# LMNS3d/SOFTX_2020_200

Hardware: AMD Instinct MI355X
Metric: nonlinear iters/sec (3D cavity Q2 128^3 BDF2) (higher is better)
Workload: dtype f64; 1 GPU; 3D lid-driven cavity Q2-Q2 128^3 transient BDF2 (BASELINE configs[2]); n_dofs=67898372, n_cells=2097152, parallelism=single

## Files before the change

include/gls_native.h:

```cpp
#ifndef GLS_NATIVE_H
#define GLS_NATIVE_H

#include <stddef.h>
#include <stdint.h>

#ifdef __cplusplus
extern "C" {
#endif

#define GLS_OK 0
#define GLS_EINVAL -1
#define GLS_EHIP -2
#define GLS_ENOMEM -3
#define GLS_ENOCONV -4
#define GLS_EIO -5
#define GLS_ECOMM -6
#define GLS_ENOTFOUND -7

enum gls_scheme {
  GLS_STEADY = 0, GLS_BDF1, GLS_BDF2, GLS_BDF3, GLS_SDIRK2, GLS_SDIRK2_1, GLS_SDIRK2_2,
  GLS_SDIRK3, GLS_SDIRK3_1, GLS_SDIRK3_2, GLS_SDIRK3_3
};

const char *gls_last_error(void);
// ... 9 lines not shown
  const int32_t *cell_vnodes;
  const int32_t *cell_pnodes;
  const double *cell_x0;
  const double *cell_h;
  const uint8_t *vnode_mask;
  double viscosity;
  int srf;
  double omega[3];
  const double *force_q;
  int map_degree;
  const double *cell_support;
} gls_mesh_desc;

typedef struct gls_ctx gls_ctx;

int gls_create(const gls_mesh_desc *desc, gls_ctx **out);
int gls_destroy(gls_ctx *ctx);
int gls_set_stream(gls_ctx *ctx, void *hip_stream);
int gls_n_dofs(const gls_ctx *ctx, int64_t *n_dofs);
int gls_quadrature_points(const gls_ctx *ctx, double *xq);
int gls_uses_brick_kernels(const gls_ctx *ctx);
int gls_set_force(gls_ctx *ctx, const double *force_q);
int gls_set_viscosity(gls_ctx *ctx, double viscosity);

int gls_set_time(gls_ctx *ctx, int scheme, const double time_steps[4]);

int gls_set_state(gls_ctx *ctx, const double *u, const double *u1, const double *u2, const double *u3);

int gls_residual(gls_ctx *ctx, double *rhs);

int gls_jacobian_apply(gls_ctx *ctx, const double *v, double *Jv);

int gls_jacobian_apply_f32(gls_ctx *ctx, const double *v, double *Jv);

int gls_set_hanging(gls_ctx *ctx, int64_t n_lines, const int64_t *dofs, const int64_t *offsets,
                    const int64_t *masters, const double *weights);

int gls_forest_bricks(const gls_ctx *ctx);

int gls_jacobian_diagonal(gls_ctx *ctx, double *diag);

int gls_residual_and_diagonal(gls_ctx *ctx, double *rhs, double *diag);

int gls_set_dirichlet(gls_ctx *ctx, int64_t n, const int64_t *dofs, const double *values);
int gls_apply_dirichlet(gls_ctx *ctx, double *x);

#define GLS_LIN_GMRES 0
#define GLS_LIN_BICGSTAB 1
#define GLS_ORTHO_GRAM 0
#define GLS_ORTHO_CGS2 1
typedef struct {
  int max_iterations;
  int restart;
  double relative_residual, minimum_residual;
  int iterations;
  double final_residual;
  int method;
  int orthogonalization;
  int true_residual;
} gls_linear_params;
int gls_solve_linear(gls_ctx *ctx, const double *rhs, double *x, gls_linear_params *prm);

typedef struct {
  int n_levels;
  gls_ctx **levels;
  int pre_smooth, post_smooth, coarse_sweeps;
  double omega;
  double coarse_omega;
  int coarse_direct;
  int mixed_precision;
  const int *level_sweeps;
  int smoother;
  int smoother_operator;
} gls_mg_params;
int gls_mg_attach(gls_ctx *ctx, const gls_mg_params *prm);
int gls_mg_attach_transfers(gls_ctx *ctx, const gls_mg_params *prm, const int64_t *const *p_off,
                            const int32_t *const *p_col, const double *const *p_w, const int64_t *const *inject);
int gls_mg_attach_replica(gls_ctx *ctx, const gls_mg_params *prm, gls_ctx *replica, const int64_t *p_off,
                          const int32_t *p_col, const double *p_w, const int64_t *inject);
int gls_apply_preconditioner(gls_ctx *ctx, const double *v, double *z);
int gls_mg_smoother_apply(gls_ctx *ctx, const double *v, double *y);
int gls_mg_transfer(gls_ctx *ctx, int level, int direction, const double *in, double *out);
int gls_mg_residual_restrict(gls_ctx *ctx, int level, const double *x, const double *b, double *bc, int *fused);
int gls_set_lattice(gls_ctx *ctx, int n1d, const int64_t *local_to_global);
int gls_mg_detach(gls_ctx *ctx);
int gls_mg_set_coarse_replica(gls_ctx *ctx, gls_ctx *replica, int64_t n_local, const int64_t *local_to_replica);
#define GLS_ILU_MAX_FILL 10
int gls_ilu_attach(gls_ctx *ctx, int fill, double athresh, double rthresh);
int gls_ilu_detach(gls_ctx *ctx);
#define GLS_ILU_ORDER_CM 0
#define GLS_ILU_ORDER_MULTICOLOR 1
int gls_ilu_set_options(gls_ctx *ctx, int ordering, int64_t block_dofs);
int gls_ilu_info(const gls_ctx *ctx, int64_t *nnz, int *n_probes);
int gls_ilu_matrix(gls_ctx *ctx, int32_t *rowp, int32_t *col, double *val);
int gls_ilu_factors(gls_ctx *ctx, int32_t *perm, int32_t *rowp, int32_t *col, double *val);
int gls_iluk_pattern(int64_t n, const int32_t *rowp, const int32_t *col, int fill, int32_t *out_rowp,
                     int32_t *out_col, int32_t *out_level, int64_t capacity, int64_t *out_nnz);
int gls_cuthill_mckee(int64_t n_nodes, const int64_t *adj_off, const int64_t *adj, const int64_t *dof_off,
                      const int64_t *dofs, int64_t *order);

#define GLS_SEC_ASSEMBLE_SYSTEM 0
#define GLS_SEC_ASSEMBLE_RHS 1
#define GLS_SEC_SETUP_ILU 2
#define GLS_SEC_SETUP_GMG 3
#define GLS_SEC_SOLVE_LINEAR 4
#define GLS_N_SECTIONS 5
int gls_section_timing(gls_ctx *ctx, int enable);
int gls_section_get(const gls_ctx *ctx, int section, double *seconds, int *calls);

#define GLS_NEWTON 0
#define GLS_SKIP_NEWTON 1
typedef struct {
  double tolerance;
  int max_iterations;
  int verbosity;
  gls_linear_params lin;
  int newton_iterations;
  int linear_iterations;
  int residual_evaluations;
  double final_residual;
  int solver;
  int skip_iterations;
  int is_initial_step;
  int force_matrix_renewal;
  int linear_failures;
} gls_newton_params;
int gls_freeze_jacobian(gls_ctx *ctx, int freeze);
int gls_newton_solve(gls_ctx *ctx, double *present, const double *u1, const double *u2, const double *u3,
                     gls_newton_params *prm);

typedef struct gls_part gls_part;
int gls_part_create(int n_cells, int nodes_per_cell, const int32_t *cell_vnodes, int n_vnodes, int rank, int world,
                    gls_part **out);
int gls_part_sizes(const gls_part *p, int64_t *cell_begin, int64_t *cell_end, int64_t *n_owned_nodes,
                   int64_t *n_local_nodes, int *n_nbrs, int64_t *n_send, int64_t *n_recv);
int gls_part_get(const gls_part *p, int32_t *local_cell_vnodes, int64_t *local_to_global, int *nbr_ranks,
                 int64_t *send_offsets, int32_t *send_nodes, int64_t *recv_offsets, int32_t *recv_nodes);
int gls_part_destroy(gls_part *p);

typedef int (*gls_exchange_fn)(void *user, int phase);
typedef int (*gls_allreduce_fn)(void *user, double *dev_buf, int n);
#define GLS_RED_BUF_MIN 256
int gls_dist_attach(gls_ctx *ctx, int64_t n_owned_nodes, int n_nbrs, const int64_t *send_offsets,
                    const int32_t *send_nodes, const int64_t *recv_offsets, const int32_t *recv_nodes, double *send_buf,
                    double *recv_buf, double *red_buf, gls_exchange_fn xchg, gls_allreduce_fn allreduce, void *user);
int gls_dist_import(gls_ctx *ctx, double *x);
#define GLS_RCCL_ID_BYTES 128
typedef struct gls_rccl gls_rccl;
int gls_rccl_unique_id(unsigned char *id_out);
int gls_rccl_create(const unsigned char *id, int rank, int world, gls_rccl **out);
int gls_rccl_destroy(gls_rccl *comm);
int gls_rccl_info(const gls_rccl *comm, int *rank, int *world);
int gls_dist_attach_rccl(gls_ctx *ctx, gls_rccl *comm, int64_t n_owned_nodes, int n_nbrs, const int *nbr_ranks,
                         const int64_t *send_offsets, const int32_t *send_nodes, const int64_t *recv_offsets,
                         const int32_t *recv_nodes);

typedef struct gls_gpart gls_gpart;
int gls_gpart_create(int dim, int k, int kp, int64_t n_cells, const int32_t *cell_vnodes, const int32_t *cell_pnodes,
                     int64_t n_vnodes, int64_t n_pnodes, int64_t n_lines, const int64_t *line_dofs,
                     const int64_t *line_offsets, const int64_t *line_masters, int rank, int world, gls_gpart **out);
int gls_gpart_sizes(const gls_gpart *p, int64_t *cell_begin, int64_t *cell_end, int64_t *n_vnodes, int64_t *n_pnodes,
                    int64_t *n_owned_vnodes, int64_t *n_owned_pnodes, int *n_nbrs, int64_t *n_send, int64_t *n_recv);
int gls_gpart_get(const gls_gpart *p, int32_t *local_cell_vnodes, int32_t *local_cell_pnodes, int64_t *vnode_l2g,
                  int64_t *pnode_l2g, int *nbr_ranks, int64_t *send_offsets, int32_t *send_dofs, int64_t *recv_offsets,
                  int32_t *recv_dofs);
int gls_gpart_map_dofs(const gls_gpart *p, int64_t n, const int64_t *global_dofs, int64_t *local_dofs);
// ... 182 lines not shown
```

softx_2020_200_amd/csrc/gls_api.cpp:

```cpp
#include <hip/hip_runtime.h>

#include <algorithm>
#include <array>
#include <chrono>
#include <cmath>
#include <cstdlib>
#include <cstdarg>
#include <cstdio>
#include <cstring>
#include <map>
#include <array>
#include <memory>
#include <string>
#include <vector>
#include <set>
#include <thread>

#include <rocblas/rocblas.h>
#include <rocsolver/rocsolver.h>
#include <rocsparse/rocsparse.h>
#include <rccl/rccl.h>

#include "../../include/gls_native.h"
#include "gls_common.hpp"
// ... 912 lines not shown
  if (c->dist.xchg(c->dist.user, 0) != 0) return set_err(GLS_ECOMM, "ghost import exchange failed");
  HIP_TRY(gls::vec_unpack_nodes(x, c->dist.recv_nodes.p, c->dist.n_recv, voff, c->dist.recv_buf, 0, c->stream));
  return GLS_OK;
}
int upload_export_order(gls_ctx::Dist &D, const int32_t *send, int64_t ns) {
  std::vector<std::pair<int32_t, int32_t>> ds;
  ds.reserve((size_t)ns);
  for (int64_t j = 0; j < ns; ++j) ds.push_back({send[j], (int32_t)j});
  std::stable_sort(ds.begin(), ds.end(), [](const std::pair<int32_t, int32_t> &a, const std::pair<int32_t, int32_t> &b) {
    return a.first < b.first;
  });
  std::vector<int32_t> au, aoff{0}, aslot;
  for (size_t t = 0; t < ds.size(); ++t) {
    if (t == 0 || ds[t].first != ds[t - 1].first) {
      if (t) aoff.push_back((int32_t)aslot.size());
      au.push_back(ds[t].first);
    }
    aslot.push_back(ds[t].second);
  }
  if (!au.empty()) aoff.push_back((int32_t)aslot.size());
  GLS_TRY(D.add_u.upload(au.data(), au.size()));
  GLS_TRY(D.add_off.upload(aoff.data(), au.empty() ? 0 : aoff.size()));
  return D.add_slot.upload(aslot.data(), aslot.size());
}
int dist_export_add(gls_ctx *c, double *y) {
  if (!c->dist.on) return GLS_OK;
  if (c->dist.dofs) {
    HIP_TRY(gls::vec_pack_dofs(y, c->dist.recv_nodes.p, c->dist.n_recv, c->dist.recv_buf, c->stream));
    if (c->dist.xchg(c->dist.user, 1) != 0) return set_err(GLS_ECOMM, "ghost export exchange failed");
    HIP_TRY(gls::vec_add_dofs_ordered(y, c->dist.add_u.p, c->dist.add_off.p, c->dist.add_slot.p, (int64_t)c->dist.add_u.n,
                                      c->dist.send_buf, c->stream));
    return GLS_OK;
  }
  const int64_t voff = 3 * (int64_t)c->n_vnodes;
  HIP_TRY(gls::vec_pack_nodes(y, c->dist.recv_nodes.p, c->dist.n_recv, voff, c->dist.recv_buf, c->stream));
  if (c->dist.xchg(c->dist.user, 1) != 0) return set_err(GLS_ECOMM, "ghost export exchange failed");
  HIP_TRY(gls::vec_add_nodes_ordered(y, c->dist.add_u.p, c->dist.add_off.p, c->dist.add_slot.p, (int64_t)c->dist.add_u.n,
                                     voff, c->dist.send_buf, c->stream));
  return GLS_OK;
}
int dist_multidot(gls_ctx *c, const double *A, int64_t lda, int nk, const double *w, double *host_out) {
  const int64_t n1 = c->dist.on ? (int64_t)c->dim * c->dist.n_owned : c->n_dofs;
  const int64_t off2 = c->dist.on ? (int64_t)c->dim * c->n_vnodes : 0;
  const int64_t n2 = c->dist.on ? c->dist.n_owned_p : 0;
  HIP_TRY(gls::vec_multidot2(A, lda, nk, w, n1, off2, n2, c->scal.p, c->work.p, c->stream));
  if (c->dist.on) {
    HIP_TRY(hipMemcpyAsync(c->dist.red_buf, c->scal.p, sizeof(double) * nk, hipMemcpyDeviceToDevice, c->stream));
    if (c->dist.allreduce(c->dist.user, c->dist.red_buf, nk) != 0) return set_err(GLS_ECOMM, "allreduce failed");
    HIP_TRY(hipMemcpyAsync(host_out, c->dist.red_buf, sizeof(double) * nk, hipMemcpyDeviceToHost, c->stream));
  } else {
    HIP_TRY(hipMemcpyAsync(host_out, c->scal.p, sizeof(double) * nk, hipMemcpyDeviceToHost, c->stream));
  }
  HIP_TRY(hipStreamSynchronize(c->stream));
  return GLS_OK;
}

int lin_f32_target(gls_ctx *c, gls::OpParams &P) {
  P.qdf = nullptr;
  if (!c->smooth_f32 || !gls::brick_fused_jacobi_supported(c->k)) return GLS_OK;
  if (c->qdata32.n != c->qdata.n) GLS_TRY(c->qdata32.alloc(c->qdata.n));
  P.qdf = c->qdata32.p;
  P.oseen = c->smooth_oseen ? 1 : 0;
  return GLS_OK;
}

int ensure_qdata(gls_ctx *c) {
  if (c->qd_valid) return GLS_OK;
  const size_t n = gls::brick_qdata_size(c->k, c->n_cells);
  if (c->qdata.n != n) GLS_TRY(c->qdata.alloc(n));
  gls::OpParams P = make_params(c, true);
  P.qd = c->qdata.p;
  GLS_TRY(lin_f32_target(c, P));
  {
    TimedLaunch t(c, 3);
    HIP_TRY(gls::launch_brick_kernel(c->k, gls::MODE_LIN, P, c->tables, c->stream));
  }
  c->qd_valid = true;
  c->qd32_valid = P.qdf != nullptr;
  c->qd32_partial = P.qdf != nullptr && P.oseen;
  return GLS_OK;
}

hipError_t slab_sum_ex(gls_ctx *g, const double *slab, const float *slabf, double *y, const uint8_t *vmask,
                       const double *jb, const double *jd, double omega, const double *rb, double *x0 = nullptr) {
  if (g->cube_nb1 > 0)
    return gls::brick_slab_sum_cube(g->k, g->cube_nb1, slab, slabf, g->n_vnodes, y, vmask, jb, jd, omega, g->stream, rb,
                                    x0);
  if (x0) return hipErrorInvalidValue;
  return gls::brick_slab_sum_ex(slab, slabf, g->sum_nodes.p, g->sum_off.p, g->sum_slots.p, (int64_t)g->sum_nodes.n,
                                g->n_vnodes, y, vmask, jb, jd, omega, g->stream, rb);
}
hipError_t slab_sum(gls_ctx *c, double *y) {
  if (c->cube_nb1 > 0)
    return gls::brick_slab_sum_cube(c->k, c->cube_nb1, c->slab.p, nullptr, c->n_vnodes, y, nullptr, nullptr, nullptr, 0.0,
                                    c->stream);
  return gls::brick_slab_sum(c->slab.p, c->sum_nodes.p, c->sum_off.p, c->sum_slots.p, (int64_t)c->sum_nodes.n,
                             c->n_vnodes, y, c->stream);
}

int rccl_exchange_on(gls_ctx *c, int phase, hipStream_t stream);

int build_brick_split(gls_ctx *c, const std::vector<char> &flag) {
  const int nvc = gls::ipow(c->k + 1, 3), nb = c->n_cells / 8;
  std::vector<int32_t> cv((size_t)c->n_cells * nvc);
  HIP_TRY(hipMemcpy(cv.data(), c->cell_vnodes.p, cv.size() * sizeof(int32_t), hipMemcpyDeviceToHost));
  std::vector<int32_t> bnd, inn;
  for (int b = 0; b < nb; ++b) {
    bool on = false;
    for (size_t e = (size_t)b * 8 * nvc; e < (size_t)(b + 1) * 8 * nvc && !on; ++e) on = flag[(size_t)cv[e]] != 0;
    (on ? bnd : inn).push_back(b);
  }
  c->split_bnd = (int)bnd.size();
  c->split_int = (int)inn.size();
  bnd.insert(bnd.end(), inn.begin(), inn.end());
  return c->split.upload(bnd.data(), std::max<size_t>(bnd.size(), 1));
}

bool split_jv_enabled(gls_ctx *c) {
  if (!c->use_brick || !c->use_qdata || c->use_colors || c->hang.on || !gls::brick_subset_supported(c->k)) return false;
  if (c->dist.on)
    return c->split.p && (c->dist.comm != nullptr || std::getenv("GLS_SPLIT_DIST"));
  const char *t = std::getenv("GLS_SPLIT_TEST");
  if (!t || std::atoi(t) < 1) return false;
  if (!c->split.p) {
    const int m = std::atoi(t), nb = c->n_cells / 8;
    std::vector<int32_t> bnd, inn;
    for (int b = 0; b < nb; ++b) (b % m == 0 ? bnd : inn).push_back(b);
    c->split_bnd = (int)bnd.size();
    c->split_int = (int)inn.size();
    bnd.insert(bnd.end(), inn.begin(), inn.end());
    if (c->split.upload(bnd.data(), std::max<size_t>(bnd.size(), 1)) != GLS_OK) return false;
  }
  return true;
}

int ensure_element_maps(gls_ctx *c) {
  if (c->ev.p || c->n_cells == 0) return GLS_OK;
  const int dim = c->dim, nv = gls::ipow(c->k + 1, dim), np = gls::ipow(c->kp + 1, dim), el = nv * dim + np;
  std::vector<int32_t> cv((size_t)c->n_cells * nv), cp;
  HIP_TRY(hipMemcpy(cv.data(), c->cell_vnodes.p, cv.size() * sizeof(int32_t), hipMemcpyDeviceToHost));
  if (c->cell_pnodes.p) {
    cp.resize((size_t)c->n_cells * np);
    HIP_TRY(hipMemcpy(cp.data(), c->cell_pnodes.p, cp.size() * sizeof(int32_t), hipMemcpyDeviceToHost));
  }
  const std::vector<int32_t> &pn = c->cell_pnodes.p ? cp : cv;
  std::vector<int64_t> voff((size_t)c->n_vnodes + 1, 0), poff((size_t)c->n_pnodes + 1, 0);
  for (int64_t e = 0; e < (int64_t)c->n_cells * nv; ++e) ++voff[(size_t)cv[(size_t)e] + 1];
  for (int64_t e = 0; e < (int64_t)c->n_cells * np; ++e) ++poff[(size_t)pn[(size_t)e] + 1];
  for (size_t i = 1; i < voff.size(); ++i) voff[i] += voff[i - 1];
  for (size_t i = 1; i < poff.size(); ++i) poff[i] += poff[i - 1];
  std::vector<int64_t> vslot((size_t)voff.back()), pslot((size_t)poff.back());
  std::vector<int64_t> vf(voff.begin(), voff.end() - 1), pf(poff.begin(), poff.end() - 1);
  for (int64_t cell = 0; cell < c->n_cells; ++cell) {
    for (int a = 0; a < nv; ++a) vslot[(size_t)vf[(size_t)cv[(size_t)(cell * nv + a)]]++] = cell * el + (int64_t)a * dim;
    for (int a = 0; a < np; ++a) pslot[(size_t)pf[(size_t)pn[(size_t)(cell * np + a)]]++] = cell * el + (int64_t)nv * dim + a;
  }
  GLS_TRY(c->ev_voff.upload(voff.data(), voff.size()));
  GLS_TRY(c->ev_vslot.upload(vslot.data(), std::max<size_t>(vslot.size(), 1)));
  GLS_TRY(c->ev_poff.upload(poff.data(), poff.size()));
  GLS_TRY(c->ev_pslot.upload(pslot.data(), std::max<size_t>(pslot.size(), 1)));
  return c->ev.alloc((size_t)c->n_cells * el);
}

int ensure_diag(gls_ctx *c);
bool cell_cache_on(const gls_ctx *c) {
  return !c->use_brick && c->n_cells > 0;
}
size_t cell_cache_size(const gls_ctx *c) {
  const int dim = c->dim;
  return (size_t)c->n_cells * (size_t)gls::ipow(c->nq1d, dim) * (size_t)(dim + dim * dim + 1 + dim);
}
// ... 667 lines not shown
  HIP_TRY(gls::vec_gather_scale_set(y, c->diag.p, v, c->con_dofs.p, (int64_t)c->con_dofs.n, c->stream));
  return GLS_OK;
}

namespace {
int ensure_qdata32(gls_ctx *g, bool full = true) {
  GLS_TRY(ensure_qdata(g));
  if (!g->qd32_valid || (full && g->qd32_partial)) {
    if (g->qdata32.n != g->qdata.n) GLS_TRY(g->qdata32.alloc(g->qdata.n));
    HIP_TRY(gls::vec_to_f32(g->qdata.p, g->qdata32.p, (int64_t)g->qdata.n, g->stream));
    g->qd32_valid = true;
    g->qd32_partial = false;
  }
  return GLS_OK;
}
bool slab_f32() { return std::getenv("GLS_SLAB_F64") == nullptr; }
bool first_sweep_fusable(gls_ctx *g) {
  const char *e = std::getenv("GLS_MG_FIRST_FUSE");
  return e && std::atoi(e) != 0 && g->smooth_f32 && g->use_brick && g->use_qdata && !g->use_colors && !g->dist.on &&
         !g->hang.on && g->k == 2 && g->cube_nb1 > 0 && g->use_slab && gls::pencil_enabled() &&
         std::getenv("GLS_MG_NO_FUSE") == nullptr;
}
int jacobian_apply_f32(gls_ctx *g, const double *v, double *y, const double *rb = nullptr, double first_omega = 0.0,
                       bool oseen = false) {
  if (!g->u) return set_err(GLS_EINVAL, "gls_set_state was not called");
  GLS_TRY(ensure_diag(g));
  GLS_TRY(ensure_qdata32(g, !oseen));
  GLS_TRY(dist_import(g, const_cast<double *>(v)));
  gls::OpParams P = make_params(g, true);
  P.qdf = g->qdata32.p;
  P.oseen = oseen ? 1 : 0;
  P.v = v;
  P.y = y;
  const bool col = g->use_colors;
  P.slab = col ? nullptr : brick_slab(g);
  const bool fuse_rb = rb && (P.slab || col) && !g->dist.on && gls::brick_fused_jacobi_supported(g->k) &&
                       std::getenv("GLS_MG_NO_FUSE") == nullptr;
  P.rb = fuse_rb ? rb : nullptr;
  P.slabf = P.slab && slab_f32() && gls::brick_fused_jacobi_supported(g->k) ? reinterpret_cast<float *>(P.slab)
                                                                             : nullptr;
  if (first_omega > 0.0) {
    if (!fuse_rb || !first_sweep_fusable(g)) return set_err(GLS_EINVAL, "fused first sweep not applicable");
    P.jx0 = const_cast<double *>(v);
    P.jd = g->diag.p;
    P.jomega = first_omega;
  }
  if (col) set_colors(g, P, y);
  if (!col && !P.slab) HIP_TRY(hipMemsetAsync(y, 0, sizeof(double) * g->n_dofs, g->stream));
  {
    TimedLaunch t(g, 4);
    HIP_TRY(gls::launch_brick_jv_f32(g->k, P, g->tables, g->stream));
  }
  if (P.slab) {
    TimedLaunch t(g, 5);
    HIP_TRY(slab_sum_ex(g, P.slab, P.slabf, y, nullptr, nullptr, P.jx0 ? g->diag.p : nullptr, P.jomega, P.rb, P.jx0));
  }
  GLS_TRY(dist_export_add(g, y));
  HIP_TRY(gls::vec_gather_scale_set(y, g->diag.p, v, g->con_dofs.p, (int64_t)g->con_dofs.n, g->stream, P.rb));
  if (rb && !fuse_rb) HIP_TRY(gls::vec_axpby(y, 1.0, rb, -1.0, g->n_dofs, g->stream));
  return GLS_OK;
}
int smoother_apply(gls_ctx *g, const double *v, double *y, const double *rb = nullptr) {
  if (g->smooth_f32 && g->use_brick && g->use_qdata) return jacobian_apply_f32(g, v, y, rb, 0.0, g->smooth_oseen);
  g->oct.f32_next = g->smooth_f32 && g->oct.on;
  const int rc = gls_jacobian_apply(g, v, y);
  g->oct.f32_next = false;
  GLS_TRY(rc);
  if (rb) HIP_TRY(gls::vec_axpby(y, 1.0, rb, -1.0, g->n_dofs, g->stream));
  return GLS_OK;
}
}
static int ensure_ilu(gls_ctx *c);
static int ilu_probe(gls_ctx *c);
static int apply_ilu(gls_ctx *c, const double *v, double *z);
namespace {
int ilu_sweep(gls_ctx *g, double *x, const double *b, double *y, double *z) {
  GLS_TRY(ensure_ilu(g));
  GLS_TRY(gls_jacobian_apply(g, x, y));
  HIP_TRY(gls::vec_axpby(y, 1.0, b, -1.0, g->n_dofs, g->stream));
  GLS_TRY(apply_ilu(g, y, z));
  HIP_TRY(gls::vec_axpy(x, 1.0, z, g->n_dofs, g->stream));
  return GLS_OK;
}
int smoother_sweep(gls_ctx *g, double *x, const double *b, double *y, double omega, double *z = nullptr) {
  if (z && g->ilu.on && !g->ilu.probe_only) return ilu_sweep(g, x, b, y, z);
  const bool nofuse = std::getenv("GLS_MG_NO_FUSE") != nullptr;
  const bool brick = g->use_brick && g->use_qdata && (g->use_colors || brick_slab(g)) && !g->dist.on &&
                     !g->hang.on && gls::brick_fused_jacobi_supported(g->k);
  if (nofuse || !brick) {
    GLS_TRY(smoother_apply(g, x, y));
    HIP_TRY(gls::mg_jacobi_update(x, b, y, g->diag.p, omega, g->n_dofs, 0, g->stream));
    return GLS_OK;
  }
  if (!g->u) return set_err(GLS_EINVAL, "gls_set_state was not called");
  GLS_TRY(ensure_diag(g));
  const bool f32 = g->smooth_f32;
  GLS_TRY(f32 ? ensure_qdata32(g, !g->smooth_oseen) : ensure_qdata(g));
  gls::OpParams P = make_params(g, true);
  P.v = x;
  P.y = x;
  P.jx = x;
  P.jb = b;
  P.jd = g->diag.p;
  P.jomega = omega;
  if (g->use_colors) {
    if (g->acc.n != (size_t)g->n_dofs) GLS_TRY(g->acc.alloc((size_t)g->n_dofs));
    set_colors(g, P, g->acc.p);
  } else {
    P.slab = brick_slab(g);
  }
  if (f32) {
    P.qdf = g->qdata32.p;
    P.oseen = g->smooth_oseen ? 1 : 0;
    P.slabf = P.slab && slab_f32() ? reinterpret_cast<float *>(P.slab) : nullptr;
    TimedLaunch t(g, 4);
    HIP_TRY(gls::launch_brick_jv_f32(g->k, P, g->tables, g->stream));
  } else {
    P.qd = g->qdata.p;
    TimedLaunch t(g, 1);
    HIP_TRY(gls::launch_brick_kernel(g->k, gls::MODE_JVQ, P, g->tables, g->stream));
  }
  if (g->use_colors) return GLS_OK;
  TimedLaunch t(g, 5);
  HIP_TRY(slab_sum_ex(g, P.slab, P.slabf, x, g->vmask.p, b, g->diag.p, omega, nullptr));
  return GLS_OK;
}
}

int gls_mg_smoother_apply(gls_ctx *c, const double *v, double *y) {
  GLS_TRY(check_ctx(c));
  if (!v || !y || v == y) return set_err(GLS_EINVAL, "v/y null or aliased");
  return smoother_apply(c, v, y);
}

int gls_jacobian_apply_f32(gls_ctx *c, const double *v, double *y) {
  GLS_TRY(check_ctx(c));
  if (!v || !y || v == y) return set_err(GLS_EINVAL, "v/y null or aliased");
  if (!(c->use_brick && c->use_qdata)) return set_err(GLS_EINVAL, "FP32 J.v needs the 3D Qk-Qk brick path");
  return jacobian_apply_f32(c, v, y);
}

int gls_set_dirichlet(gls_ctx *c, int64_t n, const int64_t *dofs, const double *vals) {
  GLS_TRY(check_ctx(c));
  if (n < 0 || (n > 0 && (!dofs || !vals))) return set_err(GLS_EINVAL, "dirichlet arrays");
  for (int64_t i = 0; i < n; ++i)
    if (dofs[i] < 0 || dofs[i] >= c->n_dofs) return set_err(GLS_EINVAL, "dirichlet dof out of range");
  HIP_TRY(hipStreamSynchronize(c->stream));
  GLS_TRY(c->dir_dofs.upload(dofs, (size_t)n));
  GLS_TRY(c->dir_vals.upload(vals, (size_t)n));
  return GLS_OK;
}

int gls_apply_dirichlet(gls_ctx *c, double *x) {
  GLS_TRY(check_ctx(c));
  HIP_TRY(gls::vec_set_indexed(x, c->dir_dofs.p, c->dir_vals.p, (int64_t)c->dir_dofs.n, c->stream));
  if (c->dist.on && c->dist.dofs) GLS_TRY(dist_import(c, x));
  if (c->hang.on)
    HIP_TRY(gls::vec_csr_gather_set(x, x, c->hang.dof.p, c->hang.off.p, c->hang.master.p, c->hang.w.p,
                                    (int64_t)c->hang.dof.n, c->stream));
  if (!c->jf.on && (x == c->u || x == c->u1 || x == c->u2 || x == c->u3)) {
    c->diag_valid = false;
    c->ilu.valid = false;
    c->qd_valid = false;
    c->cq_valid = false;
    c->mg.dirty = true;
  }
  return GLS_OK;
}

}
static int detect_oct_bricks(gls_ctx *c) {
  auto &O = c->oct;
  O = gls_ctx::Oct();
  const char *e = std::getenv("GLS_OCT_BRICKS");
  if ((e && std::atoi(e) == 0) || c->dim != 3 || c->k != 2 || c->kp != 2 || c->map_degree > 0 || c->dist.on ||
      c->cell_pnodes.p || c->host_h.empty() || !gls::pencil_enabled() || c->n_cells < 8)
    return GLS_OK;
  const int64_t nc = c->n_cells;
  std::vector<int32_t> cv((size_t)nc * 27);
  HIP_TRY(hipMemcpy(cv.data(), c->cell_vnodes.p, cv.size() * sizeof(int32_t), hipMemcpyDeviceToHost));
  std::vector<int32_t> cell0;
  std::vector<char> in((size_t)nc, 0);
  int32_t lat[125];
  for (int64_t i = 0; i + 8 <= nc;) {
    bool ok = true;
    for (int ci = 1; ci < 8 && ok; ++ci)
      for (int d = 0; d < 3; ++d) ok = ok && c->host_h[(size_t)(i + ci) * 3 + d] == c->host_h[(size_t)i * 3 + d];
    for (int t = 0; t < 125 && ok; ++t) lat[t] = -1;
    for (int ci = 0; ci < 8 && ok; ++ci) {
      const int cx = ci & 1, cy = (ci >> 1) & 1, cz = ci >> 2;
      for (int a = 0; a < 27 && ok; ++a) {
        const int X = 2 * cx + a % 3, Y = 2 * cy + (a / 3) % 3, Z = 2 * cz + a / 9;
        int32_t &slot = lat[X + 5 * (Y + 5 * Z)];
        const int32_t nd = cv[(size_t)(i + ci) * 27 + a];
        if (slot < 0) slot = nd;
        else ok = slot == nd;
      }
    }
    if (ok) {
      std::vector<int32_t> u(lat, lat + 125);
      std::sort(u.begin(), u.end());
      ok = std::adjacent_find(u.begin(), u.end()) == u.end();
    }
    if (ok) {
      cell0.push_back((int32_t)i);
      for (int ci = 0; ci < 8; ++ci) in[(size_t)(i + ci)] = 1;
      i += 8;
// ... 558 lines not shown
      HIP_TRY(gls::mg_transfer_2pass(yb, mg_box_target(c, l + 1, bc), mg.dims[l].data(), mg.dims[l + 1].data(), 1, ti,
                                     tw, tc, mg.xwork.p, s));
    else
      HIP_TRY(gls::mg_transfer3d(yb, mg_box_target(c, l + 1, bc), mg.dims[l].data(), mg.dims[l + 1].data(), ti, tw,
                                 tc, s));
  }
  GLS_TRY(mg_from_box(c, l + 1, bc));
  GLS_TRY(dist_export_add(h, bc));
  return GLS_OK;
}

bool mg_prolong_add_ok(gls_ctx *c, int l) {
  if (c->mg.csr) return false;
  return !c->mg.boxed && c->mg.taps[(size_t)l]->two_pass && std::getenv("GLS_MG_NO_FUSE") == nullptr;
}
int mg_prolong(gls_ctx *c, int l, double *xc, double *y, bool add = false) {
  auto &mg = c->mg;
  gls_ctx *h = mg.lev[(size_t)l + 1];
  hipStream_t s = c->stream;
  if (mg.csr) {
    const auto &X = *mg.xfer[(size_t)l];
    HIP_TRY(gls::vec_csr_spmv(y, xc, X.poff.p, X.pcol.p, X.pw.p, X.nf, add, s, X.plane));
    return GLS_OK;
  }
  GLS_TRY(dist_import(h, xc));
  const double *xb = mg_to_box(c, l + 1, xc, false);
  if (!xb) return set_err(GLS_EHIP, "mg box gather failed");
  {
    const auto &T = *mg.taps[(size_t)l];
    const int32_t *ti[3] = {T.pi[0].p, T.pi[1].p, T.pi[2].p}, *tc[3] = {T.pc[0].p, T.pc[1].p, T.pc[2].p};
    const double *tw[3] = {T.pw[0].p, T.pw[1].p, T.pw[2].p};
    if (T.two_pass)
      HIP_TRY(gls::mg_transfer_2pass(xb, mg_box_target(c, l, y), mg.dims[l + 1].data(), mg.dims[l].data(), 0, ti, tw,
                                     tc, mg.xwork.p, s, add ? 1 : 0));
    else if (add)
      return set_err(GLS_EINVAL, "mg_prolong: accumulate needs the two-pass transfer");
    else
      HIP_TRY(gls::mg_transfer3d(xb, mg_box_target(c, l, y), mg.dims[l + 1].data(), mg.dims[l].data(), ti, tw, tc, s));
  }
  GLS_TRY(mg_from_box(c, l, y));
  return GLS_OK;
}

bool mg_fused_restrict_ok(gls_ctx *c, int l) {
  auto &mg = c->mg;
  if (l < 0 || l + 1 >= (int)mg.lev.size() || mg.csr || mg.boxed || (size_t)l >= mg.taps.size()) return false;
  const char *e = std::getenv("GLS_MG_FUSE_TRANSFER");
  if ((e && std::atoi(e) == 0) || std::getenv("GLS_MG_NO_FUSE") != nullptr) return false;
  gls_ctx *g = mg.lev[(size_t)l], *h = mg.lev[(size_t)l + 1];
  const auto &T = *mg.taps[(size_t)l];
  const int64_t nc1 = 2 * (int64_t)g->cube_nb1 + 1;
  return T.two_pass && T.q2_brick && g->smooth_f32 && g->use_brick && g->use_qdata && !g->use_colors && !g->dist.on &&
         !g->hang.on && !g->oct.on && g->k == 2 && g->cube_nb1 > 0 && g->cube_nb1 < 1024 && g->use_slab && !g->srf &&
         gls::pencil_enabled() && gls::brick_fused_jacobi_supported(g->k) && !h->dist.on && !h->hang.on &&
         h->n_vnodes == nc1 * nc1 * nc1 && g->stream == c->stream;
}
int mg_residual_restrict_fused(gls_ctx *c, int l, double *x, const double *b, double *bc, double first_omega = 0.0) {
  gls_ctx *g = c->mg.lev[(size_t)l], *h = c->mg.lev[(size_t)l + 1];
  if (!g->u) return set_err(GLS_EINVAL, "gls_set_state was not called");
  GLS_TRY(ensure_diag(g));
  GLS_TRY(ensure_qdata32(g, !g->smooth_oseen));
  gls::OpParams P = make_params(g, true);
  P.qdf = g->qdata32.p;
  P.oseen = g->smooth_oseen ? 1 : 0;
  P.v = x;
  P.rb = b;
  P.cube_nb1 = g->cube_nb1;
  if (first_omega > 0.0) {
    P.jx0 = x;
    P.jd = g->diag.p;
    P.jomega = first_omega;
  }
  P.slab = brick_slab(g);
  if (!P.slab) return set_err(GLS_EHIP, "brick slab allocation failed");
  {
    TimedLaunch t(g, 4);
    HIP_TRY(gls::launch_pencil_jv_restrict(P, g->tables, c->stream));
  }
  TimedLaunch t(g, 5);
  HIP_TRY(gls::brick_restrict_sum_cube(g->cube_nb1, P.slab, h->n_vnodes, bc, h->vmask.p, c->stream));
  return GLS_OK;
}

bool coarse_graph_eligible(gls_ctx *c, gls_ctx *g, const double *b, const double *x) {
  const int l = (int)c->mg.lev.size() - 1;
  return !c->mg.cgraph_failed && !c->mg.boxed && !g->dist.on && !g->hang.on && g->use_brick && g->use_qdata &&
         brick_slab(g) && gls::brick_fused_jacobi_supported(g->k) && g->stream == c->stream &&
         b == mgbuf(c, l, MB_B) && x == mgbuf(c, l, MB_X) && std::getenv("GLS_MG_NO_FUSE") == nullptr &&
         std::getenv("GLS_MG_GRAPH") != nullptr;
}
}
static std::vector<unsigned char> coarse_graph_key(gls_ctx *g, const double *b, const double *x, const double *y,
                                                   int pre, double om) {
  const gls::OpParams P = make_params(g);
  const void *ptrs[7] = {b, x, y, g->diag.p, g->qdata.p, g->qdata32.p, brick_slab(g)};
  const int64_t ints[4] = {pre, g->n_dofs, (int64_t)g->smooth_f32, (int64_t)slab_f32()};
  std::vector<unsigned char> k(sizeof(P) + sizeof(ptrs) + sizeof(ints) + sizeof(om));
  unsigned char *o = k.data();
  std::memcpy(o, &P, sizeof(P));
  std::memcpy(o += sizeof(P), ptrs, sizeof(ptrs));
  std::memcpy(o += sizeof(ptrs), ints, sizeof(ints));
  std::memcpy(o + sizeof(ints), &om, sizeof(om));
  return k;
}
extern "C" {
int coarse_graph_capture(gls_ctx *c, gls_ctx *g, const double *b, double *x, double *y, int pre, double om) {
  auto &mg = c->mg;
  hipStream_t s = c->stream;
  GLS_TRY(ensure_diag(g));
  GLS_TRY(g->smooth_f32 ? ensure_qdata32(g, !g->smooth_oseen) : ensure_qdata(g));
  if (g->use_colors && g->acc.n != (size_t)g->n_dofs) GLS_TRY(g->acc.alloc((size_t)g->n_dofs));
  const bool tim = g->timing;
  g->timing = false;
  hipGraph_t gr = nullptr;
  int rc = GLS_OK;
  hipError_t e = hipStreamBeginCapture(s, hipStreamCaptureModeThreadLocal);
  if (e == hipSuccess) {
    if (hipError_t e1 = gls::mg_jacobi_update(x, b, nullptr, g->diag.p, om, g->n_dofs, 1, s); e1 != hipSuccess)
      e = e1;
    for (int it = 1; it < pre && rc == GLS_OK && e == hipSuccess; ++it) rc = smoother_sweep(g, x, b, y, om);
    const hipError_t e2 = hipStreamEndCapture(s, &gr);
    if (e == hipSuccess) e = e2;
  }
  g->timing = tim;
  hipGraphExec_t ex = nullptr;
  if (rc == GLS_OK && e == hipSuccess && gr) e = hipGraphInstantiate(&ex, gr, nullptr, nullptr, 0);
  if (gr) (void)hipGraphDestroy(gr);
  if (rc != GLS_OK || e != hipSuccess || !ex) {
    (void)hipGetLastError();
    if (ex) (void)hipGraphExecDestroy(ex);
    mg.cgraph_failed = true;
    if (std::getenv("GLS_MG_VERBOSE")) std::printf("mg: coarse graph capture refused (%s)\n", hipGetErrorString(e));
    return GLS_OK;
  }
  mg.cgraph.h = ex;
  mg.cgraph_key = coarse_graph_key(g, b, x, y, pre, om);
  return GLS_OK;
}

int dist_allreduce_vector(gls_ctx *c, double *v, int64_t n) {
  auto &D = c->dist;
  if (!D.on) return GLS_OK;
  if (D.comm) {
    if (D.allreduce(D.user, v, (int)n) != 0) return set_err(GLS_ECOMM, "vector all-reduce failed");
    return GLS_OK;
  }
  hipStream_t s = c->stream;
  for (int64_t o = 0; o < n; o += GLS_RED_BUF_MIN) {
    const int len = (int)std::min<int64_t>(GLS_RED_BUF_MIN, n - o);
    HIP_TRY(hipMemcpyAsync(D.red_buf, v + o, sizeof(double) * len, hipMemcpyDeviceToDevice, s));
    if (D.allreduce(D.user, D.red_buf, len) != 0) return set_err(GLS_ECOMM, "vector all-reduce failed");
    HIP_TRY(hipMemcpyAsync(v + o, D.red_buf, sizeof(double) * len, hipMemcpyDeviceToDevice, s));
  }
  return GLS_OK;
}
int rep2_inject(gls_ctx *c, const double *loc, double *glob) {
  auto &mg = c->mg;
  const int64_t ng = mg.rep2->n_dofs, ni = (int64_t)mg.r2inj_c.n;
  HIP_TRY(gls::vec_fill(glob, ng, 0.0, c->stream));
  if (ni) {
    HIP_TRY(gls::vec_pack_dofs(loc, mg.r2inj_f.p, ni, mg.rep_tmp.p, c->stream));
    HIP_TRY(gls::vec_unpack_dofs(glob, mg.r2inj_c.p, ni, mg.rep_tmp.p, c->stream));
  }
  return dist_allreduce_vector(c, glob, ng);
}
int mg_vcycle_rep2(gls_ctx *c, const double *b, double *x) {
// ... 89 lines not shown
        HIP_TRY(gls::vec_to_f32(bb, mg.x32.p, n, c->stream));
        HIP_TRY(gls::dense_lu_solve_f32(mg.probe32.p, (int)n, mg.x32.p, c->stream, bl, bu));
        if (mg.lu32_refine) {
          const double one = 1.0, mone = -1.0;
          double *r = mg.chk32.p, *x0 = mg.chk32.p + n;
          HIP_TRY(gls::vec_from_f32(mg.x32.p, x0, n, c->stream));
          HIP_TRY(gls::vec_copy(r, bb, n, c->stream));
          if (rocblas_set_stream(mg.blas, c->stream) != rocblas_status_success ||
              rocblas_dgemv(mg.blas, rocblas_operation_none, (rocblas_int)n, (rocblas_int)n, &mone, mg.probe.p,
                            (rocblas_int)n, x0, 1, &one, r, 1) != rocblas_status_success)
            return set_err(GLS_EHIP, "rocblas_dgemv failed");
          HIP_TRY(gls::vec_to_f32(r, mg.x32.p, n, c->stream));
          HIP_TRY(gls::dense_lu_solve_f32(mg.probe32.p, (int)n, mg.x32.p, c->stream, bl, bu));
          HIP_TRY(gls::vec_from_f32(mg.x32.p, xx, n, c->stream));
          HIP_TRY(gls::vec_axpy(xx, 1.0, x0, n, c->stream));
        } else {
          HIP_TRY(gls::vec_from_f32(mg.x32.p, xx, n, c->stream));
        }
      } else {
        const float one = 1.0f, zero = 0.0f;
        HIP_TRY(gls::vec_to_f32(bb, mg.b32.p, n, c->stream));
        if (rocblas_set_stream(mg.blas, c->stream) != rocblas_status_success ||
            rocblas_sgemv(mg.blas, rocblas_operation_none, (rocblas_int)n, (rocblas_int)n, &one, mg.probe32.p,
                          (rocblas_int)n, mg.b32.p, 1, &zero, mg.x32.p, 1) != rocblas_status_success)
          return set_err(GLS_EHIP, "rocblas_sgemv failed");
        HIP_TRY(gls::vec_from_f32(mg.x32.p, xx, n, c->stream));
      }
      if (mg.lu_cm) HIP_TRY(gls::vec_permute(x, mg.lu_tmp.p, g->ilu.perm.p, n, 1, c->stream));
      HIP_TRY(hipMemsetAsync(x + (int64_t)g->dim * g->n_vnodes, 0, sizeof(double), c->stream));
      return GLS_OK;
    }
    if (mg.lu) {
      const double one = 1.0, zero = 0.0;
      if (rocblas_set_stream(mg.blas, c->stream) != rocblas_status_success ||
          rocblas_dgemv(mg.blas, rocblas_operation_none, (rocblas_int)n, (rocblas_int)n, &one, mg.probe.p,
                        (rocblas_int)n, b, 1, &zero, x, 1) != rocblas_status_success)
        return set_err(GLS_EHIP, "rocblas_dgemv failed");
    } else {
      HIP_TRY(gls::mg_dense_apply(mg.aug.p, (int)n, b, x, c->stream));
    }
    return GLS_OK;
  }
  const int pre = l == L - 1 ? mg.csweeps : mg.lpre[(size_t)l];
  const double om = l == L - 1 ? mg.comega : mg.omega;
  if (l == L - 1 && l > 0 && pre > 1 && coarse_graph_eligible(c, g, b, x)) {
    GLS_TRY(ensure_diag(g));
    GLS_TRY(g->smooth_f32 ? ensure_qdata32(g, !g->smooth_oseen) : ensure_qdata(g));
    if (mg.cgraph.h && mg.cgraph_key != coarse_graph_key(g, b, x, y, pre, om)) mg.cgraph.reset();
    if (!mg.cgraph.h) GLS_TRY(coarse_graph_capture(c, g, b, x, y, pre, om));
    if (mg.cgraph.h) {
      HIP_TRY(hipGraphLaunch(mg.cgraph.h, s));
      return GLS_OK;
    }
  }
  const bool first_fused = pre == 1 && l < L - 1 && first_sweep_fusable(g);
  double *zs = mg.ilu_smooth && g->ilu.on && !g->ilu.probe_only ? mgbuf(c, l, MB_BOX) : nullptr;
  if (pre > 0 && !first_fused && zs) {
    GLS_TRY(ensure_ilu(g));
    GLS_TRY(apply_ilu(g, b, x));
    for (int it = 1; it < pre; ++it) GLS_TRY(smoother_sweep(g, x, b, y, om, zs));
  } else if (pre > 0 && !first_fused) {
    HIP_TRY(gls::mg_jacobi_update(x, b, nullptr, d, om, n, 1, s));
    for (int it = 1; it < pre; ++it) GLS_TRY(smoother_sweep(g, x, b, y, om));
  } else if (pre == 0) {
    HIP_TRY(gls::vec_fill(x, n, 0.0, s));
  }
  if (l == L - 1) return GLS_OK;
  gls_ctx *h = mg.lev[l + 1];
  double *bc = mgbuf(c, l + 1, MB_B), *xc = mgbuf(c, l + 1, MB_X);
  if (pre > 0 && mg_fused_restrict_ok(c, l)) {
    GLS_TRY(mg_residual_restrict_fused(c, l, x, b, bc, first_fused ? om : 0.0));
  } else {
    if (first_fused) {
      GLS_TRY(jacobian_apply_f32(g, x, y, b, om, g->smooth_oseen));
    } else if (pre > 0) {
      GLS_TRY(smoother_apply(g, x, y, b));
    } else {
      HIP_TRY(gls::vec_copy(y, b, n, s));
    }
    GLS_TRY(mg_restrict(c, l, y, bc));
    HIP_TRY(gls::vec_set_indexed(bc, h->con_dofs.p, nullptr, (int64_t)h->con_dofs.n, s));
  }
  GLS_TRY(mg_vcycle(c, l + 1, bc, xc));
  if (mg_prolong_add_ok(c, l)) {
    GLS_TRY(mg_prolong(c, l, xc, x, true));
  } else {
    GLS_TRY(mg_prolong(c, l, xc, y));
    HIP_TRY(gls::vec_set_indexed(y, g->con_dofs.p, nullptr, (int64_t)g->con_dofs.n, s));
    HIP_TRY(gls::vec_axpy(x, 1.0, y, n, s));
  }
  for (int it = 0; it < mg.lpost[(size_t)l]; ++it) GLS_TRY(smoother_sweep(g, x, b, y, mg.omega, zs));
  return GLS_OK;
}

#define RS_TRY(x)                                                                        \
  do {                                                                                   \
    const rocsparse_status rs_ = (x);                                                    \
    if (rs_ != rocsparse_status_success) return set_err(GLS_EHIP, "%s: rocsparse status %d", #x, (int)rs_); \
  } while (0)

static int ilu_probe_batched(gls_ctx *c) {
  auto &I = c->ilu;
  const int64_t n = c->n_dofs;
  hipStream_t s = c->stream;
  if (!c->u) return set_err(GLS_EINVAL, "gls_set_state was not called");
  GLS_TRY(ensure_element_maps(c));
  if (c->con_dofs.n) GLS_TRY(ensure_diag(c));
  const int dim = c->dim, nv = gls::ipow(c->k + 1, dim), np = gls::ipow(c->kp + 1, dim);
  const int64_t el = (int64_t)nv * dim + np, evs = (int64_t)c->n_cells * el;
  const char *bs = std::getenv("GLS_ILU_PROBE_BATCH");
  const int64_t budget = (int64_t)1 << 31;
  int B = bs ? std::atoi(bs) : (int)std::min<int64_t>(I.n_probes, std::max<int64_t>(1, budget / (8 * (3 * n + evs))));
  B = std::max(1, std::min(B, I.n_probes));
  if (I.bV.n < (size_t)B * n) {
    GLS_TRY(I.bV.alloc((size_t)B * n));
    GLS_TRY(I.bY.alloc((size_t)B * n));
  }
  if (c->hang.on && I.bC.n < (size_t)B * n) GLS_TRY(I.bC.alloc((size_t)B * n));
  if (c->bev.n < (size_t)B * evs) GLS_TRY(c->bev.alloc((size_t)B * evs));
  const int cb = gls::cell_kernel_cells_per_block(dim, c->k, c->nq1d, true), nblk = (c->n_cells + cb - 1) / cb;
  if (c->bact.n < (size_t)B * nblk) GLS_TRY(c->bact.alloc((size_t)B * nblk));
  if (I.fill > 0) HIP_TRY(gls::vec_fill(I.val.p, I.nnz, 0.0, s));
  const char *wl_env = std::getenv("GLS_ILU_PROBE_LIST");
  const bool wl_on = !(wl_env && wl_env[0] == '0');
  const bool use_list = wl_on && !I.woff.empty() && I.wB == B && I.wnblk == nblk;
  const bool record = wl_on && !use_list;
  bool cq_probe = use_list && cell_cache_on(c) && !c->oct.on;
  if (cq_probe) {
    GLS_TRY(ensure_diag(c));
    cq_probe = c->cq_valid && c->cq.n == cell_cache_size(c);
  }
  std::vector<int32_t> hlist;
  std::vector<int64_t> hoff;
  std::vector<uint8_t> hact;
  if (record) {
    GLS_TRY(I.wact.alloc((size_t)I.n_probes * nblk));
    hoff.push_back(0);
  }
  for (int p0 = 0; p0 < I.n_probes; p0 += B) {
    const int nb = std::min(B, I.n_probes - p0);
    HIP_TRY(gls::vec_fill(I.bV.p, (int64_t)nb * n, 0.0, s));
    const int64_t d0 = I.pdoff[(size_t)p0], d1 = I.pdoff[(size_t)(p0 + nb)];
    HIP_TRY(gls::probe_set_batched(I.bV.p, n, I.pdofs.p + d0, I.pdpid.p + d0, p0, d1 - d0, s));
    const double *Cv = I.bV.p;
    if (c->hang.on) {
      HIP_TRY(gls::vec_copy(I.bC.p, I.bV.p, (int64_t)nb * n, s));
      HIP_TRY(gls::vec_csr_gather_set_b(I.bC.p, c->hang.dof.p, c->hang.ooff.p, c->hang.omaster.p, c->hang.ow.p,
                                        (int64_t)c->hang.dof.n, nb, n, s));
      Cv = I.bC.p;
    }
    gls::OpParams P = make_params(c, true);
    P.v = Cv;
    P.y = I.bY.p;
    P.hmask = c->hang.on ? c->hang.hmask.p : nullptr;
    P.ev = c->bev.p;
    P.bv_stride = n;
    P.bev_stride = evs;
    P.n_probe = nb;
    const int chunk = p0 / B;
    P.bact = use_list ? I.wact.p + (size_t)p0 * nblk : c->bact.p;
    if (use_list) {
      P.work = I.wlist.p + 2 * I.woff[(size_t)chunk];
      P.n_work = (int)(I.woff[(size_t)chunk + 1] - I.woff[(size_t)chunk]);
      if (cq_probe) {
        P.cq = c->cq.p;
        P.cq_mode = 2;
      }
    }
    if (!use_list || P.n_work > 0) {
      TimedLaunch t(c, (int)gls::MODE_JV);
      HIP_TRY(gls::launch_cell_kernel(c->dim, c->k, c->kp, c->nq1d, gls::MODE_JV, P, c->tables, s));
    }
    if (record) {
      HIP_TRY(hipMemcpyAsync(I.wact.p + (size_t)p0 * nblk, c->bact.p, (size_t)nb * nblk, hipMemcpyDeviceToDevice, s));
// ... 84 lines not shown
                               I.mc_map.n ? I.mc_map.p : nullptr, I.mc_compact, I.rdiag.p, s));
  else
    RS_TRY(rocsparse_dcsrilu0(I.h, m, nnz, I.dA, I.val.p, I.rowp32.p, I.col.p, I.info, rocsparse_solve_policy_auto, I.work.p));
  I.valid = true;
  if (verbose) {
    const auto t2 = now();
    rocsparse_int zp = -1;
    const rocsparse_status st = I.h ? rocsparse_csrilu0_zero_pivot(I.h, I.info, &zp) : rocsparse_status_success;
    GLS_TRY(apply_ilu(c, I.ybuf.p, I.ybuf.p == nullptr ? nullptr : c->tmp1.p ? c->tmp1.p : I.ybuf.p));
    const auto t3 = now();
    std::printf("ilu: %d probes %.2f ms, csrilu0 %.2f ms (zero pivot status %d at %d), one apply %.3f ms\n", I.n_probes,
                std::chrono::duration<double, std::milli>(t1 - t0).count(),
                std::chrono::duration<double, std::milli>(t2 - t1).count(), (int)st, (int)zp,
                std::chrono::duration<double, std::milli>(t3 - t2).count());
  }
  return GLS_OK;
}
static int apply_ilu(gls_ctx *c, const double *v, double *z) {
  auto &I = c->ilu;
  const rocsparse_int m = (rocsparse_int)c->n_dofs, nnz = (rocsparse_int)I.nnz;
  const double one = 1.0;
  if (I.h) RS_TRY(rocsparse_set_stream(I.h, c->stream));
  HIP_TRY(gls::vec_permute(I.vbuf.p, v, I.perm.p, c->n_dofs, 0, c->stream));
  if (I.mc_solve) {
    HIP_TRY(gls::ilu_mc_solve(I.mc_desc.p, I.mc_cg.data(), (int)I.mc_cg.size() - 1, I.col.p, I.val.p, I.vbuf.p,
                              I.tbuf.p, I.vbuf.p, I.mc_wl.data(), I.mc_wu.data(), c->stream));
    HIP_TRY(gls::vec_permute(z, I.vbuf.p, I.perm.p, c->n_dofs, 1, c->stream));
    return GLS_OK;
  }
  RS_TRY(rocsparse_dcsrsv_solve(I.h, rocsparse_operation_none, m, nnz, &one, I.dL, I.val.p, I.rowp32.p, I.col.p, I.info,
                                I.vbuf.p, I.tbuf.p, rocsparse_solve_policy_auto, I.work.p));
  RS_TRY(rocsparse_dcsrsv_solve(I.h, rocsparse_operation_none, m, nnz, &one, I.dU, I.val.p, I.rowp32.p, I.col.p, I.info,
                                I.tbuf.p, I.vbuf.p, rocsparse_solve_policy_auto, I.work.p));
  HIP_TRY(gls::vec_permute(z, I.vbuf.p, I.perm.p, c->n_dofs, 1, c->stream));
  return GLS_OK;
}

int apply_prec(gls_ctx *c, const double *v, double *z) {
  if (c->mg.on && c->mg.rep_csr) return mg_vcycle_rep2(c, v, z);
  if (c->mg.on) return mg_vcycle(c, 0, v, z);
  if (c->ilu.on && !c->ilu.probe_only) return apply_ilu(c, v, z);
  HIP_TRY(gls::vec_div(z, v, c->diag.p, c->n_dofs, c->stream));
  return GLS_OK;
}
}

int gls_apply_preconditioner(gls_ctx *c, const double *v, double *z) {
  GLS_TRY(check_ctx(c));
  if (!v || !z || v == z) return set_err(GLS_EINVAL, "v/z null or aliased");
  GLS_TRY(ensure_diag(c));
  if (c->mg.on) GLS_TRY(mg_prepare(c));
  GLS_TRY(ensure_ilu(c));
  return apply_prec(c, v, z);
}

int gls_mg_transfer(gls_ctx *c, int level, int direction, const double *in, double *out) {
  GLS_TRY(check_ctx(c));
  auto &mg = c->mg;
  if (!mg.on) return set_err(GLS_EINVAL, "gls_mg_transfer: no multigrid attached");
  if (level < 0 || level + 1 >= (int)mg.lev.size() || (direction != 0 && direction != 1) || !in || !out || in == out)
    return set_err(GLS_EINVAL, "gls_mg_transfer: bad level / direction / pointers");
  if (direction == 0) return mg_restrict(c, level, in, out);
  double *xc = mgbuf(c, level + 1, MB_X);
  HIP_TRY(gls::vec_copy(xc, in, mg.lev[(size_t)level + 1]->n_dofs, c->stream));
  return mg_prolong(c, level, xc, out);
}

int gls_mg_residual_restrict(gls_ctx *c, int level, const double *x, const double *b, double *bc, int *fused) {
  GLS_TRY(check_ctx(c));
  auto &mg = c->mg;
  if (!mg.on) return set_err(GLS_EINVAL, "gls_mg_residual_restrict: no multigrid attached");
  if (level < 0 || level + 1 >= (int)mg.lev.size() || !x || !b || !bc)
    return set_err(GLS_EINVAL, "gls_mg_residual_restrict: bad level / pointers");
  GLS_TRY(mg_prepare(c));
  const bool f = mg_fused_restrict_ok(c, level);
  if (fused) *fused = f ? 1 : 0;
  if (f) return mg_residual_restrict_fused(c, level, const_cast<double *>(x), b, bc);
  gls_ctx *g = mg.lev[(size_t)level], *h = mg.lev[(size_t)level + 1];
  double *y = mgbuf(c, level, MB_Y);
  GLS_TRY(smoother_apply(g, x, y, b));
  GLS_TRY(mg_restrict(c, level, y, bc));
  HIP_TRY(gls::vec_set_indexed(bc, h->con_dofs.p, nullptr, (int64_t)h->con_dofs.n, c->stream));
  return GLS_OK;
}

namespace {
int build_face_neighbours(gls_ctx *c) {
  const int dim = c->dim, k = c->k, nv = gls::ipow(k + 1, dim);
  std::vector<int32_t> cn((size_t)c->n_cells * nv);
  if (!cn.empty() && hipMemcpy(cn.data(), c->cell_vnodes.p, cn.size() * sizeof(int32_t), hipMemcpyDeviceToHost) != hipSuccess)
    return set_err(GLS_EHIP, "cell map download failed");
  std::map<std::array<int32_t, 4>, std::pair<int, int>> open;
  std::vector<int32_t> nbr((size_t)c->n_cells * 2 * dim, -1);
  for (int cell = 0; cell < c->n_cells; ++cell)
    for (int d = 0; d < dim; ++d)
      for (int sd = 0; sd < 2; ++sd) {
        std::array<int32_t, 4> key = {-1, -1, -1, -1};
        int nk = 0;
        for (int v = 0; v < (1 << dim); ++v) {
          if (((v >> d) & 1) != sd) continue;
          int a = 0, st = 1;
          for (int e = 0; e < dim; ++e, st *= k + 1) a += ((v >> e) & 1) * k * st;
          key[nk++] = cn[(size_t)cell * nv + a];
        }
        std::sort(key.begin(), key.begin() + nk);
        auto it = open.find(key);
        if (it == open.end()) {
          open.emplace(key, std::make_pair(cell, 2 * d + sd));
        } else {
          nbr[(size_t)cell * 2 * dim + 2 * d + sd] = it->second.first;
          nbr[(size_t)it->second.first * 2 * dim + it->second.second] = cell;
          open.erase(it);
        }
      }
  return c->face_nbr.upload(nbr.data(), nbr.size());
}

gls::KellyTables kelly_tables(int m, int nq) {
  gls::KellyTables T;
  std::memset(&T, 0, sizeof(T));
  double xq[gls::kMaxQ1D], wq[gls::kMaxQ1D], xn[gls::kMaxNodes1D];
  gauss_points(nq, xq, wq);
  lobatto_points(m, xn);
  T.nq = nq;
  for (int a = 0; a <= m; ++a) {
    double v, dd, s2;
    for (int q = 0; q < nq; ++q) {
      lagrange_1d(m, xn, a, xq[q], v, dd, s2);
      T.V[q][a] = v;
    }
    lagrange_1d(m, xn, a, 0.0, v, dd, s2);
    T.De[0][a] = dd;
    lagrange_1d(m, xn, a, 1.0, v, dd, s2);
    T.De[1][a] = dd;
  }
  for (int q = 0; q < nq; ++q) {
    T.w[q] = wq[q];
    T.xq[q] = xq[q];
  }
  for (int a = 0; a <= m; ++a) T.xn[a] = xn[a];
  return T;
}
}

int gls_kelly_estimate(gls_ctx *c, const double *sol, int variable, double *eta) {
  GLS_TRY(check_ctx(c));
  if (!sol || !eta || (variable != 0 && variable != 1)) return set_err(GLS_EINVAL, "gls_kelly_estimate: bad arguments");
  if (c->hang.on) return set_err(GLS_EINVAL, "gls_kelly_estimate: conforming meshes only (no hanging nodes)");
  if (c->map_degree > 0) return set_err(GLS_EINVAL, "gls_kelly_estimate: axis-aligned box cells only");
  if (c->nq1d + 1 > gls::kMaxQ1D) return set_err(GLS_EINVAL, "gls_kelly_estimate: face rule too large");
  if (!c->face_nbr.p && c->n_cells > 0) GLS_TRY(build_face_neighbours(c));
  const bool pres = variable == 1;
  const int m = pres ? c->kp : c->k;
  const int32_t *nodes = pres && c->cell_pnodes.p ? c->cell_pnodes.p : c->cell_vnodes.p;
  const gls::KellyTables T = kelly_tables(m, c->nq1d + 1);
  HIP_TRY(gls::launch_kelly(c->dim, m, nodes, c->face_nbr.p, c->geo.p, sol, c->n_cells, pres ? 1 : c->dim,
                            pres ? (int64_t)c->dim * c->n_vnodes : 0, pres ? 1 : c->dim, T, eta, c->stream));
  return GLS_OK;
}

int gls_kelly_estimate_faces(gls_ctx *c, const double *sol, int variable, int64_t n_faces, const int32_t *fa,
                             const int32_t *fb, const int32_t *fdir, const double *rect_a, const double *rect_b,
                             double *eta) {
  GLS_TRY(check_ctx(c));
  if (!sol || !eta || (variable != 0 && variable != 1) || n_faces < 0 || (n_faces > 0 && (!fa || !fb || !fdir || !rect_a || !rect_b)))
    return set_err(GLS_EINVAL, "gls_kelly_estimate_faces: bad arguments");
// ... 2389 lines not shown
```

softx_2020_200_amd/csrc/gls_brick_common.hpp:

```cpp
#pragma once
#include "gls_common.hpp"

namespace gls {

__device__ __forceinline__ int xcd_swizzle(int orig, int n) {
  const int q = n / 8, r = n % 8, x = orig % 8;
  return (x < r ? x * (q + 1) : r * (q + 1) + (x - r) * q) + orig / 8;
}

template <int BN>
__device__ __forceinline__ int bnd_index(int X, int Y, int Z) {
  constexpr int I = BN - 2;
  const int n = X + BN * (Y + BN * Z);
  int before = min(max(Z - 1, 0), I) * I * I;
  if (Z >= 1 && Z <= I) {
    before += min(max(Y - 1, 0), I) * I;
    if (Y >= 1 && Y <= I) before += min(max(X - 1, 0), I);
  }
  return n - before;
}

__device__ __forceinline__ void wave_sync() {
#ifdef GLS_WAVE_SYNC_DRAIN
  asm volatile("s_waitcnt lgkmcnt(0)" ::: "memory");
#else
  asm volatile("" ::: "memory");
#endif
  __builtin_amdgcn_wave_barrier();
}

constexpr int kQdpRow = 54;
constexpr int kQdpTriple = 4 * 3 * kQData * kQdpRow;
__device__ __forceinline__ int64_t qdp_base(int brick, int ci, int q) {
  const int cw = (brick % 3) * 8 + ci, w = cw / 6, c = cw % 6;
  const int qx = q % 3, qy = (q / 3) % 3, qz = q / 9;
  return (int64_t)(brick / 3) * kQdpTriple + ((w * 3 + qz) * kQData) * kQdpRow + 9 * c + 3 * qy + qx;
}

}
```

softx_2020_200_amd/csrc/gls_brick_kernels.hip:

```cpp
#include "gls_brick_common.hpp"
#include "gls_common.hpp"
#include "gls_launch.hpp"

#include <algorithm>
#include <cstdlib>
#include <type_traits>

#ifndef GLS_ABL
#define GLS_ABL 0
#endif
#ifndef GLS_ROWS_REG
#define GLS_ROWS_REG 1
#endif
#ifndef GLS_BRICK_WAVES_PER_EU
#define GLS_BRICK_WAVES_PER_EU 4
#endif
#ifndef GLS_BRICK_WPE_F32
#define GLS_BRICK_WPE_F32 6
#endif

#ifndef GLS_QD_LITE
#define GLS_QD_LITE 0
#endif

// ... 1000 lines not shown
  double s[4] = {0., 0., 0., 0.};
#if GLS_SLAB_INFLIGHT
  const int j0 = off[i], cnt = off[i + 1] - j0;
  int sl[8];
#pragma unroll
  for (int t = 0; t < 8; ++t) sl[t] = t < cnt ? slots[j0 + t] : 0;
  double e[8][4];
#pragma unroll
  for (int t = 0; t < 8; ++t)
    if (t < cnt) SlabQuad<S>::load(slab + (int64_t)sl[t] * 4, e[t][0], e[t][1], e[t][2], e[t][3]);
#pragma unroll
  for (int t = 0; t < 8; ++t)
    if (t < cnt) {
      s[0] += e[t][0];
      s[1] += e[t][1];
      s[2] += e[t][2];
      s[3] += e[t][3];
    }
  for (int j = j0 + 8; j < j0 + cnt; ++j) {
    double a, b, c, d;
    SlabQuad<S>::load(slab + (int64_t)slots[j] * 4, a, b, c, d);
    s[0] += a;
    s[1] += b;
    s[2] += c;
    s[3] += d;
  }
#else
  for (int j = off[i]; j < off[i + 1]; ++j) {
    double a, b, c, d;
    SlabQuad<S>::load(slab + (int64_t)slots[j] * 4, a, b, c, d);
    s[0] += a;
    s[1] += b;
    s[2] += c;
    s[3] += d;
  }
#endif
  const int64_t node = nodes[i];
  const int64_t gi[4] = {node * 3, node * 3 + 1, node * 3 + 2, voff + node};
  if constexpr (J) {
    const unsigned m = vmask ? vmask[node] : 0u;
#pragma unroll
    for (int f = 0; f < 4; ++f) {
      const double x = y[gi[f]], dd = jd[gi[f]];
      y[gi[f]] = x + jomega * (jb[gi[f]] - ((f < 3 && ((m >> f) & 1u)) ? dd * x : s[f])) / dd;
    }
  } else {
    if (rb) {
#pragma unroll
      for (int f = 0; f < 4; ++f) y[gi[f]] = rb[gi[f]] - s[f];
    } else {
#pragma unroll
      for (int f = 0; f < 4; ++f) y[gi[f]] = s[f];
    }
  }
}
hipError_t brick_slab_sum(const double *slab, const int32_t *nodes, const int32_t *off, const int32_t *slots,
                          int64_t n_sum, int64_t n_vnodes, double *y, hipStream_t s) {
  if (n_sum <= 0) return hipSuccess;
  hipLaunchKernelGGL((k_slab_sum<double, false>), dim3((unsigned)((n_sum + 255) / 256)), dim3(256), 0, s, slab, nodes,
                     off, slots, n_sum, 3 * n_vnodes, y, nullptr, nullptr, nullptr, 0.0, nullptr);
  return hipGetLastError();
}
hipError_t brick_slab_sum_ex(const double *slab, const float *slabf, const int32_t *nodes, const int32_t *off,
                             const int32_t *slots, int64_t n_sum, int64_t n_vnodes, double *y, const uint8_t *vmask,
                             const double *jb, const double *jd, double jomega, hipStream_t s, const double *rb) {
  if (n_sum <= 0) return hipSuccess;
  const dim3 g((unsigned)((n_sum + 255) / 256)), b(256);
  const int64_t voff = 3 * n_vnodes;
  if (slabf) {
    if (jb) hipLaunchKernelGGL((k_slab_sum<float, true>), g, b, 0, s, slabf, nodes, off, slots, n_sum, voff, y, vmask, jb, jd, jomega, rb);
    else hipLaunchKernelGGL((k_slab_sum<float, false>), g, b, 0, s, slabf, nodes, off, slots, n_sum, voff, y, vmask, jb, jd, jomega, rb);
  } else {
    if (jb) hipLaunchKernelGGL((k_slab_sum<double, true>), g, b, 0, s, slab, nodes, off, slots, n_sum, voff, y, vmask, jb, jd, jomega, rb);
    else hipLaunchKernelGGL((k_slab_sum<double, false>), g, b, 0, s, slab, nodes, off, slots, n_sum, voff, y, vmask, jb, jd, jomega, rb);
  }
  return hipGetLastError();
}
__device__ __forceinline__ uint32_t morton3(uint32_t x, uint32_t y, uint32_t z) {
  uint32_t m = 0;
  for (int b = 0; b < 10; ++b)
    m |= (((x >> b) & 1u) << (3 * b)) | (((y >> b) & 1u) << (3 * b + 1)) | (((z >> b) & 1u) << (3 * b + 2));
  return m;
}
template <typename S, bool J, int K>
__global__ void __launch_bounds__(256) k_slab_sum_cube(const S *__restrict__ slab, int nb1, int64_t voff,
                                                       double *__restrict__ y, const uint8_t *__restrict__ vmask,
                                                       const double *__restrict__ jb, const double *__restrict__ jd,
                                                       double jomega, const double *__restrict__ rb,
                                                       double *__restrict__ x0) {
  constexpr int BN = 2 * K + 1, P2 = 2 * K, NBND = BN * BN * BN - (BN - 2) * (BN - 2) * (BN - 2);
  const int NX = P2 * nb1 + 1;
  int bx = blockIdx.x, Z = blockIdx.y;
  if (GLS_SLAB_XCD) {
    const int lin = xcd_swizzle((int)(blockIdx.x + gridDim.x * blockIdx.y), (int)(gridDim.x * gridDim.y));
    bx = lin % (int)gridDim.x;
    Z = lin / (int)gridDim.x;
  }
  const bool zs = Z % P2 == 0;
  const int64_t t = (int64_t)bx * blockDim.x + threadIdx.x;
  int X, Y;
  const int ns = nb1 + 1;
  if (zs) {
    if (t >= (int64_t)NX * NX) return;
    X = (int)(t % NX);
    Y = (int)(t / NX);
  } else {
    const int64_t full = (int64_t)ns * NX, sparse = (int64_t)(NX - ns) * ns;
    if (t >= full + sparse) return;
    if (t < full) {
      X = (int)(t % NX);
      Y = (int)(t / NX) * P2;
    } else {
      const int64_t u = t - full;
      const int r = (int)(u / ns);
      X = (int)(u % ns) * P2;
      Y = (r / (P2 - 1)) * P2 + 1 + r % (P2 - 1);
    }
  }
  int bc[3][2], lc[3][2], nc[3];
  const int co[3] = {X, Y, Z};
#pragma unroll
  for (int d = 0; d < 3; ++d) {
    const int x = co[d];
    if (x % P2 == 0 && x > 0 && x < NX - 1) {
      nc[d] = 2;
      bc[d][0] = x / P2 - 1;
      lc[d][0] = P2;
      bc[d][1] = x / P2;
      lc[d][1] = 0;
    } else {
      nc[d] = 1;
      bc[d][0] = min(x / P2, nb1 - 1);
      lc[d][0] = x - P2 * bc[d][0];
      bc[d][1] = bc[d][0];
      lc[d][1] = lc[d][0];
    }
  }
  int64_t sl[8];
  int cnt = 0;
#pragma unroll
  for (int k = 0; k < 2; ++k)
#pragma unroll
    for (int j = 0; j < 2; ++j)
#pragma unroll
      for (int i = 0; i < 2; ++i) {
        const bool on = i < nc[0] && j < nc[1] && k < nc[2];
        const int64_t s = (int64_t)morton3(bc[0][i], bc[1][j], bc[2][k]) * NBND + bnd_index<BN>(lc[0][i], lc[1][j], lc[2][k]);
        sl[i + 2 * j + 4 * k] = on ? s : INT64_MAX;
        cnt += on;
      }
  auto cs = [&](int a, int b) {
    const int64_t lo = min(sl[a], sl[b]), hi = max(sl[a], sl[b]);
    sl[a] = lo;
    sl[b] = hi;
  };
  cs(0, 1); cs(2, 3); cs(4, 5); cs(6, 7);
  cs(0, 2); cs(1, 3); cs(4, 6); cs(5, 7);
  cs(1, 2); cs(5, 6); cs(0, 4); cs(3, 7);
  cs(1, 5); cs(2, 6);
  cs(1, 4); cs(3, 6);
  cs(2, 4); cs(3, 5);
  cs(3, 4);
  double e[8][4];
#pragma unroll
  for (int q = 0; q < 8; ++q)
    if (q < cnt) SlabQuad<S>::load(slab + sl[q] * 4, e[q][0], e[q][1], e[q][2], e[q][3]);
  double s[4] = {0., 0., 0., 0.};
#pragma unroll
  for (int q = 0; q < 8; ++q)
    if (q < cnt) {
      s[0] += e[q][0];
      s[1] += e[q][1];
      s[2] += e[q][2];
      s[3] += e[q][3];
    }
  const int64_t node = X + (int64_t)NX * (Y + (int64_t)NX * Z);
  const int64_t gi[4] = {node * 3, node * 3 + 1, node * 3 + 2, voff + node};
  if constexpr (J) {
    const unsigned m = vmask ? vmask[node] : 0u;
#pragma unroll
    for (int f = 0; f < 4; ++f) {
      const double x = y[gi[f]], dd = jd[gi[f]];
      y[gi[f]] = x + jomega * (jb[gi[f]] - ((f < 3 && ((m >> f) & 1u)) ? dd * x : s[f])) / dd;
    }
  } else if (rb) {
#pragma unroll
    for (int f = 0; f < 4; ++f) y[gi[f]] = rb[gi[f]] - s[f];
    if (x0) {
#pragma unroll
      for (int f = 0; f < 4; ++f) x0[gi[f]] = 0.0 + jomega * rb[gi[f]] / jd[gi[f]];
    }
  } else {
#pragma unroll
    for (int f = 0; f < 4; ++f) y[gi[f]] = s[f];
  }
}
hipError_t brick_slab_sum_cube(int k, int nb1, const double *slab, const float *slabf, int64_t n_vnodes, double *y,
                               const uint8_t *vmask, const double *jb, const double *jd, double jomega, hipStream_t s,
                               const double *rb, double *x0) {
  if (nb1 <= 0 || (k != 1 && k != 2)) return hipErrorInvalidValue;
  if (x0 && (!rb || !jd || jb)) return hipErrorInvalidValue;
  const int NX = 2 * k * nb1 + 1;
  const dim3 g((unsigned)(((int64_t)NX * NX + 255) / 256), (unsigned)NX), b(256);
  const int64_t voff = 3 * n_vnodes;
#define GLS_SLAB_CUBE(KK)                                                                                                   \
  if (slabf) {                                                                                                              \
    if (jb) hipLaunchKernelGGL((k_slab_sum_cube<float, true, KK>), g, b, 0, s, slabf, nb1, voff, y, vmask, jb, jd, jomega, rb, x0);  \
    else hipLaunchKernelGGL((k_slab_sum_cube<float, false, KK>), g, b, 0, s, slabf, nb1, voff, y, vmask, jb, jd, jomega, rb, x0);   \
  } else {                                                                                                                  \
    if (jb) hipLaunchKernelGGL((k_slab_sum_cube<double, true, KK>), g, b, 0, s, slab, nb1, voff, y, vmask, jb, jd, jomega, rb, x0); \
    else hipLaunchKernelGGL((k_slab_sum_cube<double, false, KK>), g, b, 0, s, slab, nb1, voff, y, vmask, jb, jd, jomega, rb, x0);  \
  }
  if (k == 1) {
    GLS_SLAB_CUBE(1)
  } else {
    GLS_SLAB_CUBE(2)
  }
#undef GLS_SLAB_CUBE
  return hipGetLastError();
}

__global__ void __launch_bounds__(256) k_restrict_sum_cube(const double *__restrict__ ev, int nb1, int64_t voff,
                                                           double *__restrict__ bc, const uint8_t *__restrict__ vmask) {
  const int NX = 2 * nb1 + 1;
  int bx = blockIdx.x, Z = blockIdx.y;
  if (GLS_SLAB_XCD) {
    const int lin = xcd_swizzle((int)(blockIdx.x + gridDim.x * blockIdx.y), (int)(gridDim.x * gridDim.y));
    bx = lin % (int)gridDim.x;
    Z = lin / (int)gridDim.x;
  }
  const int64_t t = (int64_t)bx * blockDim.x + threadIdx.x;
  if (t >= (int64_t)NX * NX) return;
  const int X = (int)(t % NX), Y = (int)(t / NX);
  int bcd[3][2], lc[3][2], nc[3];
  const int co[3] = {X, Y, Z};
#pragma unroll
  for (int d = 0; d < 3; ++d) {
    const int x = co[d];
    if (x % 2 == 0 && x > 0 && x < NX - 1) {
      nc[d] = 2;
      bcd[d][0] = x / 2 - 1;
      lc[d][0] = 2;
      bcd[d][1] = x / 2;
      lc[d][1] = 0;
    } else {
      nc[d] = 1;
      bcd[d][0] = min(x / 2, nb1 - 1);
      lc[d][0] = x - 2 * bcd[d][0];
      bcd[d][1] = bcd[d][0];
      lc[d][1] = lc[d][0];
    }
  }
  int64_t sl[8];
  int cnt = 0;
#pragma unroll
  for (int k = 0; k < 2; ++k)
#pragma unroll
    for (int j = 0; j < 2; ++j)
#pragma unroll
      for (int i = 0; i < 2; ++i) {
        const bool on = i < nc[0] && j < nc[1] && k < nc[2];
        const int64_t s = (int64_t)morton3(bcd[0][i], bcd[1][j], bcd[2][k]) * 27 + lc[0][i] + 3 * (lc[1][j] + 3 * lc[2][k]);
        sl[i + 2 * j + 4 * k] = on ? s : INT64_MAX;
        cnt += on;
      }
  auto cs = [&](int a, int b) {
    const int64_t lo = min(sl[a], sl[b]), hi = max(sl[a], sl[b]);
    sl[a] = lo;
    sl[b] = hi;
  };
  cs(0, 1); cs(2, 3); cs(4, 5); cs(6, 7);
  cs(0, 2); cs(1, 3); cs(4, 6); cs(5, 7);
  cs(1, 2); cs(5, 6); cs(0, 4); cs(3, 7);
  cs(1, 5); cs(2, 6);
  cs(1, 4); cs(3, 6);
  cs(2, 4); cs(3, 5);
  cs(3, 4);
  double e[8][4];
#pragma unroll
  for (int q = 0; q < 8; ++q)
    if (q < cnt) SlabQuad<double>::load(ev + sl[q] * 4, e[q][0], e[q][1], e[q][2], e[q][3]);
  double s[4] = {0., 0., 0., 0.};
#pragma unroll
  for (int q = 0; q < 8; ++q)
    if (q < cnt) {
      s[0] += e[q][0];
      s[1] += e[q][1];
      s[2] += e[q][2];
      s[3] += e[q][3];
    }
  const int64_t node = X + (int64_t)NX * (Y + (int64_t)NX * Z);
  const unsigned m = vmask ? vmask[node] : 0u;
  bc[node * 3] = (m & 1u) ? 0.0 : s[0];
  bc[node * 3 + 1] = (m & 2u) ? 0.0 : s[1];
// ... 35 lines not shown
```

softx_2020_200_amd/csrc/gls_brick_pencil.hip:

```cpp
#include "gls_brick_common.hpp"
#include "gls_common.hpp"
#include "gls_launch.hpp"

#include <cstdlib>
#include <type_traits>

#ifndef GLS_PENCIL_WPE64
#define GLS_PENCIL_WPE64 2
#endif
#ifndef GLS_PENCIL_PIPE
#define GLS_PENCIL_PIPE 1
#endif
#ifndef GLS_PENCIL_NT
#define GLS_PENCIL_NT 0
#endif
#ifndef GLS_PENCIL_WPE32
#define GLS_PENCIL_WPE32 4
#endif

namespace gls {

template <typename Real, bool JV>
struct PencilCfg {
  static constexpr int K1 = 3, N3 = 27, BN = 5, BN3 = 125, BN3P = 128, NBND = 98;
  static constexpr int CPW = 6, WAVES = 4, THREADS = 256, CPG = 24, BPG = 3;
  static constexpr bool F64 = sizeof(Real) == 8;
  static constexpr int SY = 5, SZ = 25, FB = JV ? (F64 ? 131 : 129) : 128;
  static constexpr int XS = JV ? (F64 ? 12 : 16) : 10, XA = 3 * XS;
  static constexpr int ZS = JV ? (F64 ? 12 : 10) : 10, ZAZ = 3, ZA = 3 * ZS, WB = 3 * ZA, WAZ = 9,
                       WA = 28;
  static constexpr int CSF = 3 * XA, CSB = WB + 2 * WA;
  static constexpr int CS0 = CSF > CSB ? CSF : CSB;
  static constexpr int CS = JV ? (F64 ? 190 : 164) : CS0 + 4;
  static constexpr int NO = 4;
  static constexpr int OF = 27, OC = JV ? 123 : NO * OF;
  static_assert(CS >= CS0 && OC >= NO * OF && FB >= 4 * SZ + 4 * SY + 5, "pencil LDS layout");
};

constexpr int pencil_fields(int mode) { return mode == MODE_JVQ ? 4 : 7; }
template <typename Real, bool JV>
size_t pencil_lds_bytes_t(int mode) {
  using C = PencilCfg<Real, JV>;
  return sizeof(Real) * ((size_t)C::BPG * pencil_fields(mode) * C::FB + (size_t)C::WAVES * C::CPW * C::CS +
                         (size_t)C::CPG * C::OC) +
         sizeof(int) * (size_t)C::BPG * C::BN3P;
}
template <typename Real>
size_t pencil_lds_bytes(int mode) {
  return mode == MODE_JVQ ? pencil_lds_bytes_t<Real, true>(mode) : pencil_lds_bytes_t<Real, false>(mode);
}

template <typename Real>
struct PencilTab {
  Real V[3][3], D[3][3], S[3][3], w[3], xi[3];
};

template <typename Real, int MODE, bool GEN, bool FOREST = false, bool OS = false, bool RST = false>
__global__ void __launch_bounds__(256, (std::is_same<Real, float>::value ? GLS_PENCIL_WPE32 : GLS_PENCIL_WPE64))
    gls_pencil_kernel(const OpParams P, const PencilTab<Real> T) {
  static_assert(!OS || (MODE == MODE_JVQ && std::is_same<Real, float>::value), "Oseen operator: FP32 J.v only");
  static_assert(!RST || (MODE == MODE_JVQ && std::is_same<Real, float>::value && !FOREST), "restriction: FP32 J.v on the cube");
  using C = PencilCfg<Real, MODE == MODE_JVQ>;
  constexpr bool RL = MODE == MODE_RESLIN, RES = MODE == MODE_RESIDUAL || RL, LIN = MODE == MODE_LIN || RL;
  constexpr bool ST = RES || LIN;
  constexpr int BN = C::BN, BN3 = C::BN3, BN3P = C::BN3P, NF = pencil_fields(MODE);
  extern __shared__ __attribute__((aligned(16))) char smem_raw[];
  constexpr int FB = C::FB, SY = C::SY, SZ = C::SZ;
  Real *const sB = reinterpret_cast<Real *>(smem_raw);
  Real *const sS = sB + C::BPG * NF * FB;
  constexpr int CS = C::CS;
  Real *const sO = sS + C::WAVES * C::CPW * CS;
  int *const sNode = reinterpret_cast<int *>(sO + C::CPG * C::OC);
  __shared__ Real sRow[3 * 16];

  const int tid = threadIdx.x, lane = tid & 63, wave = tid >> 6;
  const int n_bricks = P.n_cells / 8;
  const int32_t *const subset = (std::is_same<Real, double>::value || FOREST) ? P.subset : nullptr;
  const int n_items = subset ? P.subset_n : n_bricks;
  const int n_groups = (n_items + 2) / 3;
  const int g = xcd_swizzle((int)blockIdx.x, n_groups);
  const int nbg = min(3, n_items - 3 * g);
  auto brick_of = [&](int bi) { return subset ? subset[3 * g + bi] : 3 * g + bi; };
  auto cell0 = [&](int b) -> int64_t { return P.brick_cell0 ? (int64_t)P.brick_cell0[b] : (int64_t)b * 8; };
  const int64_t voff = (int64_t)3 * P.n_vnodes;

  if (tid < 48) {
    const int mat = tid >> 4, r = (tid >> 2) & 3, cc = tid & 3;
    Real v = 0;
    if (r < 3 && cc < 3) v = mat == 0 ? T.V[r][cc] : mat == 1 ? T.D[r][cc] : T.S[r][cc];
    sRow[tid] = v;
  }
  const bool act = lane < 9 * C::CPW;
  const int c = act ? lane / 9 : 0, rr = act ? lane % 9 : 0, pa = rr % 3, pb = rr / 3;
  const int cw = wave * C::CPW + c, bi = cw >> 3, ci = cw & 7;
  const bool valid = act && bi < nbg;
  const int brick = brick_of(valid ? bi : 0);
  const int cx = ci & 1, cy = (ci >> 1) & 1, cz = ci >> 2;
  const int64_t gcell = cell0(brick) + (valid ? ci : 0);
  const Real hx = (Real)P.geo[gcell * 4 + 0], hy = (Real)P.geo[gcell * 4 + 1], hz = (Real)P.geo[gcell * 4 + 2];
  const Real ihx = Real(1) / hx, ihy = Real(1) / hy, ihz = Real(1) / hz;
  const Real wxx = ihx * ihx, wyy = ihy * ihy, wzz = ihz * ihz;
  Real *const cellS = sS + (wave * C::CPW + c) * CS;
  const Real *qrow = nullptr;
  if constexpr (!ST) {
    const Real *base = std::is_same<Real, double>::value ? reinterpret_cast<const Real *>(P.qd)
                                                          : reinterpret_cast<const Real *>(P.qdf);
    qrow = base + qdp_base(brick, valid ? ci : 0, pa + 3 * pb);
  }
  for (int t = tid; t < C::BPG * BN3; t += C::THREADS) {
    const int bi = t / BN3, n = t % BN3;
    if (bi >= nbg) break;
    const int brick = brick_of(bi);
    const int X = n % BN, Y = (n / BN) % BN, Z = n / (BN * BN);
    const int cx = min(X / 2, 1), cy = min(Y / 2, 1), cz = min(Z / 2, 1);
    const int a = (X - 2 * cx) + 3 * ((Y - 2 * cy) + 3 * (Z - 2 * cz));
    const int node = P.cell_vnodes[(cell0(brick) + cx + 2 * cy + 4 * cz) * 27 + a];
    const int64_t i3 = (int64_t)node * 3;
    Real *b = sB + bi * NF * FB + X + SY * Y + SZ * Z;
    if constexpr (ST) {
      double h[3] = {0., 0., 0.};
#pragma unroll
      for (int cc = 0; cc < 3; ++cc) {
        if (P.n_hist > 0) h[cc] += P.alpha[1] * P.h1[i3 + cc];
        if (P.n_hist > 1) h[cc] += P.alpha[2] * P.h2[i3 + cc];
        if (P.n_hist > 2) h[cc] += P.alpha[3] * P.h3[i3 + cc];
      }
      b[0] = (Real)P.u[i3];
      b[FB] = (Real)P.u[i3 + 1];
      b[2 * FB] = (Real)P.u[i3 + 2];
      b[3 * FB] = (Real)P.u[voff + node];
      b[4 * FB] = (Real)h[0];
      b[5 * FB] = (Real)h[1];
      b[6 * FB] = (Real)h[2];
    } else {
      double v0, v1, v2, vp;
      if (P.jx0) {
        v0 = 0.0 + P.jomega * P.rb[i3] / P.jd[i3];
        v1 = 0.0 + P.jomega * P.rb[i3 + 1] / P.jd[i3 + 1];
        v2 = 0.0 + P.jomega * P.rb[i3 + 2] / P.jd[i3 + 2];
        vp = 0.0 + P.jomega * P.rb[voff + node] / P.jd[voff + node];
      } else {
        v0 = P.v[i3], v1 = P.v[i3 + 1], v2 = P.v[i3 + 2], vp = P.v[voff + node];
      }
      const unsigned m = P.vmask ? P.vmask[node] : 0u;
      b[0] = (m & 1u) ? Real(0) : (Real)v0;
      b[FB] = (m & 2u) ? Real(0) : (Real)v1;
      b[2 * FB] = (m & 4u) ? Real(0) : (Real)v2;
      b[3 * FB] = (Real)vp;
    }
    sNode[bi * BN3P + n] = node;
  }
  __syncthreads();


  auto xsweep = [&](int f, int kind, int base) {
    const bool grad = kind >= 1, vel = kind == 2;
    const Real *F = sB + (bi < 3 ? bi : 0) * NF * FB + f * FB + 2 * cx + SY * (2 * cy + pa) + SZ * (2 * cz + pb);
    const Real f0 = F[0], f1 = F[1], f2 = F[2];
    Real *const X = cellS + base;
#pragma unroll
    for (int qx = 0; qx < 3; ++qx) {
      const Real xb = T.V[qx][0] * f0 + T.V[qx][1] * f1 + T.V[qx][2] * f2;
      const Real xd = grad ? T.D[qx][0] * f0 + T.D[qx][1] * f1 + T.D[qx][2] * f2 : Real(0);
      const int o = qx * C::XS + pa + 3 * pb;
      const Real xs = vel ? T.S[qx][0] * f0 + T.S[qx][1] * f1 + T.S[qx][2] * f2 : Real(0);
      if (act) {
        X[0 * C::XA + o] = xb;
        if (grad) X[1 * C::XA + o] = xd;
        if (vel) X[2 * C::XA + o] = xs;
      }
    }
  };
  auto ysweep = [&](int kind, int base, Real (&BB)[3], Real (&BD)[3], Real (&DB)[3], Real (&LL)[3]) {
    const bool grad = kind >= 1, vel = kind == 2;
    const Real *rowp = sRow + pb * 4;
    const Real v0 = rowp[0], v1 = rowp[1], v2 = rowp[2];
    const Real d0 = rowp[16], d1 = rowp[17], d2 = rowp[18];
    const Real s0 = rowp[32], s1 = rowp[33], s2 = rowp[34];
    Real xb[9], xd[9], xs[9];
    const Real *sl = cellS + base + pa * C::XS;
#pragma unroll
    for (int e = 0; e < 9; ++e) {
      xb[e] = sl[e];
      if (grad) xd[e] = sl[C::XA + e];
      if (vel) xs[e] = sl[2 * C::XA + e];
    }
#pragma unroll
    for (int k = 0; k < 3; ++k) {
      const Real b0 = xb[3 * k], b1 = xb[3 * k + 1], b2 = xb[3 * k + 2];
      BB[k] = v0 * b0 + v1 * b1 + v2 * b2;
      if (grad) {
        BD[k] = d0 * b0 + d1 * b1 + d2 * b2;
// ... 28 lines not shown
      for (int m = 0; m < 3; ++m)
#pragma unroll
        for (int az = 0; az < 3; ++az) cellS[zb + m * C::ZA + pa * C::ZS + C::ZAZ * az + pb] = Z[m][az];
    }
  };
  auto bwd_w = [&](int zb, int wb) {
    const Real *Zs = cellS + zb;
    Real *Ws = cellS + wb;
    Real z[3][3];
#pragma unroll
    for (int m = 0; m < 3; ++m)
#pragma unroll
      for (int qy = 0; qy < 3; ++qy) z[m][qy] = Zs[m * C::ZA + pa * C::ZS + C::ZAZ * pb + qy];
#pragma unroll
    for (int ay = 0; ay < 3; ++ay) {
      const Real w0 = T.V[0][ay] * z[0][0] + T.V[1][ay] * z[0][1] + T.V[2][ay] * z[0][2] +
                      (T.D[0][ay] * z[2][0] + T.D[1][ay] * z[2][1] + T.D[2][ay] * z[2][2]);
      const Real w1 = T.V[0][ay] * z[1][0] + T.V[1][ay] * z[1][1] + T.V[2][ay] * z[1][2];
      if (act) {
        Ws[0 * C::WA + C::WAZ * pb + 3 * ay + pa] = w0;
        Ws[1 * C::WA + C::WAZ * pb + 3 * ay + pa] = w1;
      }
    }
  };
  auto bwd_out = [&](int f, int wb) {
    const Real *Ws = cellS + wb;
    Real w0[3], w1[3];
#pragma unroll
    for (int qx = 0; qx < 3; ++qx) {
      w0[qx] = Ws[C::WAZ * pb + 3 * pa + qx];
      w1[qx] = Ws[C::WA + C::WAZ * pb + 3 * pa + qx];
    }
    if (valid) {
#pragma unroll
      for (int ax = 0; ax < 3; ++ax)
        outc[f * C::OF + 9 * pb + 3 * pa + ax] =
            T.V[0][ax] * w0[0] + T.V[1][ax] * w0[1] + T.V[2][ax] * w0[2] +
            (T.D[0][ax] * w1[0] + T.D[1][ax] * w1[1] + T.D[2][ax] * w1[2]);
    }
  };
  auto backward = [&](int f, const Real (&Z)[3][3]) {
    bwd_z(Z, 0);
    wave_sync();
    bwd_w(0, C::WB);
    wave_sync();
    bwd_out(f, C::WB);
    wave_sync();
  };

  auto reduce_scatter = [&](double *yo, double *slo, bool fused) {
    for (int t = tid; t < C::BPG * BN3; t += C::THREADS) {
      const int rb_ = t / BN3, n = t % BN3;
      if (rb_ >= nbg) break;
      const int bk = brick_of(rb_);
      const int Xn = n % BN, Yn = (n / BN) % BN, Zn = n / (BN * BN);
      Real s[4] = {0, 0, 0, 0};
#pragma unroll
      for (int kz = 0; kz < 2; ++kz) {
        const int az = Zn - 2 * kz;
        if (az < 0 || az > 2) continue;
#pragma unroll
        for (int ky = 0; ky < 2; ++ky) {
          const int ay = Yn - 2 * ky;
          if (ay < 0 || ay > 2) continue;
#pragma unroll
          for (int kx = 0; kx < 2; ++kx) {
            const int ax = Xn - 2 * kx;
            if (ax < 0 || ax > 2) continue;
            const Real *o = sO + (rb_ * 8 + kx + 2 * ky + 4 * kz) * C::OC + ax + 3 * (ay + 3 * az);
#pragma unroll
            for (int f = 0; f < 4; ++f) s[f] += o[f * C::OF];
          }
        }
      }
      const int node = sNode[rb_ * BN3P + n];
      const int64_t gi[4] = {(int64_t)node * 3, (int64_t)node * 3 + 1, (int64_t)node * 3 + 2, voff + node};
      const bool interior = Xn > 0 && Xn < BN - 1 && Yn > 0 && Yn < BN - 1 && Zn > 0 && Zn < BN - 1;
      if (interior) {
        if (fused && P.jx) {
          const unsigned m = P.vmask ? P.vmask[node] : 0u;
#pragma unroll
          for (int f = 0; f < 4; ++f) {
            const bool con = f < 3 && ((m >> f) & 1u);
            const double x = P.jx[gi[f]], dd = P.jd[gi[f]];
            P.jx[gi[f]] = x + P.jomega * (P.jb[gi[f]] - (con ? dd * x : (double)s[f])) / dd;
          }
        } else if (fused && P.rb) {
#pragma unroll
          for (int f = 0; f < 4; ++f) yo[gi[f]] = P.rb[gi[f]] - (double)s[f];
          if (P.jx0) {
#pragma unroll
            for (int f = 0; f < 4; ++f) P.jx0[gi[f]] = 0.0 + P.jomega * P.rb[gi[f]] / P.jd[gi[f]];
          }
        } else {
#pragma unroll
          for (int f = 0; f < 4; ++f) yo[gi[f]] = s[f];
        }
      } else {
        const int64_t si = ((int64_t)bk * C::NBND + bnd_index<BN>(Xn, Yn, Zn)) * 4;
        if (fused && std::is_same<Real, float>::value && P.slabf) {
          typedef float f4 __attribute__((ext_vector_type(4)));
          *reinterpret_cast<f4 *>(P.slabf + si) = f4{(float)s[0], (float)s[1], (float)s[2], (float)s[3]};
        } else {
          typedef double d2 __attribute__((ext_vector_type(2)));
          *reinterpret_cast<d2 *>(slo + si) = d2{(double)s[0], (double)s[1]};
          *reinterpret_cast<d2 *>(slo + si + 2) = d2{(double)s[2], (double)s[3]};
        }
      }
    }
  };

  auto write_ev = [&]() {
    for (int t = tid; t < nbg * 8 * 27; t += C::THREADS) {
      const int rb_ = t / 216, r = t - rb_ * 216, ci_ = r / 27, a = r - ci_ * 27;
      const Real *o = sO + (rb_ * 8 + ci_) * C::OC + a;
      double *e = P.ev + (cell0(brick_of(rb_)) + ci_) * 108;
      e[a * 3] = (double)o[0];
      e[a * 3 + 1] = (double)o[C::OF];
      e[a * 3 + 2] = (double)o[2 * C::OF];
      e[81 + a] = (double)o[3 * C::OF];
    }
  };

  auto restrict_store = [&]() {
    auto r53 = [](double r0, double r1, double r2, double r3, double r4, double &c0, double &c1, double &c2) {
      c0 = r0 + (0.375 * r1 - 0.125 * r3);
      c1 = r2 + 0.75 * (r1 + r3);
      c2 = r4 + (0.375 * r3 - 0.125 * r1);
    };
    auto compact3 = [](unsigned v) {
      v &= 0x09249249u;
      v = (v ^ (v >> 2)) & 0x030c30c3u;
      v = (v ^ (v >> 4)) & 0x0300f00fu;
      v = (v ^ (v >> 8)) & 0xff0000ffu;
      return (int)((v ^ (v >> 16)) & 0x3ffu);
    };
    static_assert((C::BPG * NF * FB + C::WAVES * C::CPW * CS) % 2 == 0 && C::BPG * NF * FB + C::WAVES * C::CPW * CS >= 2 * (C::BPG * 4 * (BN3 + 45)) &&
                      C::CPG * C::OC >= 2 * C::BPG * 4 * 75, "restriction scratch in LDS");
    double *const dR = reinterpret_cast<double *>(sB), *const dY = dR + C::BPG * 4 * BN3;
    double *const dX = reinterpret_cast<double *>(sO);
    for (int t = tid; t < C::BPG * BN3; t += C::THREADS) {
      const int rb_ = t / BN3, n = t % BN3;
      if (rb_ >= nbg) break;
      const int bk = brick_of(rb_);
      const int Xn = n % BN, Yn = (n / BN) % BN, Zn = n / (BN * BN);
      Real s[4] = {0, 0, 0, 0};
#pragma unroll
      for (int kz = 0; kz < 2; ++kz) {
        const int az = Zn - 2 * kz;
        if (az < 0 || az > 2) continue;
#pragma unroll
        for (int ky = 0; ky < 2; ++ky) {
          const int ay = Yn - 2 * ky;
          if (ay < 0 || ay > 2) continue;
#pragma unroll
          for (int kx = 0; kx < 2; ++kx) {
            const int ax = Xn - 2 * kx;
            if (ax < 0 || ax > 2) continue;
            const Real *o = sO + (rb_ * 8 + kx + 2 * ky + 4 * kz) * C::OC + ax + 3 * (ay + 3 * az);
#pragma unroll
            for (int f = 0; f < 4; ++f) s[f] += o[f * C::OF];
          }
        }
      }
      const int node = sNode[rb_ * BN3P + n];
      const int top = P.cube_nb1 - 1;
      const bool own = (Xn < BN - 1 || compact3((unsigned)bk) == top) && (Yn < BN - 1 || compact3((unsigned)bk >> 1) == top) &&
                       (Zn < BN - 1 || compact3((unsigned)bk >> 2) == top);
      const unsigned m = P.vmask ? P.vmask[node] : 0u;
      double r[4] = {-(double)s[0], -(double)s[1], -(double)s[2], -(double)s[3]};
      if (own) {
        const int64_t gi[4] = {(int64_t)node * 3, (int64_t)node * 3 + 1, (int64_t)node * 3 + 2, voff + node};
#pragma unroll
        for (int f = 0; f < 4; ++f) r[f] = P.rb[gi[f]] - (double)s[f];
        if (P.jx0) {
#pragma unroll
          for (int f = 0; f < 4; ++f) P.jx0[gi[f]] = 0.0 + P.jomega * P.rb[gi[f]] / P.jd[gi[f]];
        }
      }
#pragma unroll
      for (int f = 0; f < 4; ++f) dR[(rb_ * 4 + f) * BN3 + n] = (f < 3 && ((m >> f) & 1u)) ? 0.0 : r[f];
    }
    __syncthreads();
    for (int t = tid; t < nbg * 4 * 25; t += C::THREADS) {
      const int bf = t / 25, yz = t - bf * 25;
      const double *r = dR + bf * BN3 + BN * yz;
      double *o = dX + bf * 75 + 3 * yz;
      r53(r[0], r[1], r[2], r[3], r[4], o[0], o[1], o[2]);
    }
    __syncthreads();
    for (int t = tid; t < nbg * 4 * 15; t += C::THREADS) {
      const int bf = t / 15, zx = t - bf * 15, Z = zx / 3, cx_ = zx - 3 * Z;
      const double *r = dX + bf * 75 + 15 * Z + cx_;
      double *o = dY + bf * 45 + 9 * Z + cx_;
      r53(r[0], r[3], r[6], r[9], r[12], o[0], o[3], o[6]);
    }
    __syncthreads();
    for (int t = tid; t < nbg * 9; t += C::THREADS) {
      const int rb_ = t / 9, xy = t - rb_ * 9;
      double cv[4][3];
#pragma unroll
      for (int f = 0; f < 4; ++f) {
        const double *r = dY + (rb_ * 4 + f) * 45 + xy;
        r53(r[0], r[9], r[18], r[27], r[36], cv[f][0], cv[f][1], cv[f][2]);
      }
      typedef double d2 __attribute__((ext_vector_type(2)));
      d2 *e = reinterpret_cast<d2 *>(P.slab + ((int64_t)brick_of(rb_) * 27 + xy) * 4);
#pragma unroll
      for (int cz_ = 0; cz_ < 3; ++cz_) {
        e[18 * cz_] = d2{cv[0][cz_], cv[1][cz_]};
        e[18 * cz_ + 1] = d2{cv[2][cz_], cv[3][cz_]};
      }
    }
  };

  if constexpr (ST) {
    Real uq[3][3], Ttq[3][3], pq[3], gp[3][3];
    {
      Real dz[3];
#pragma unroll
      for (int cc = 0; cc < 3; ++cc) {
        Real bb[3], hb[3];
        forward(cc, 0, bb, dz, dz, dz);
        forward(4 + cc, 0, hb, dz, dz, dz);
#pragma unroll
        for (int qz = 0; qz < 3; ++qz) {
          uq[cc][qz] = zval(bb, qz);
          Ttq[cc][qz] = (Real)P.alpha[0] * uq[cc][qz] + zval(hb, qz);
        }
      }
      Real pb_[3], pbd[3], pdb[3];
      forward(3, 1, pb_, pbd, pdb, dz);
#pragma unroll
      for (int qz = 0; qz < 3; ++qz) {
        pq[qz] = zval(pb_, qz);
        gp[0][qz] = zval(pdb, qz) * ihx;
        gp[1][qz] = zval(pbd, qz) * ihy;
        gp[2][qz] = zder(pb_, qz) * ihz;
      }
    }
    const Real hst = (Real)P.geo[gcell * 4 + 3];
    Real tauq[3];
#pragma unroll
    for (int qz = 0; qz < 3; ++qz) {
      const Real un2 = uq[0][qz] * uq[0][qz] + uq[1][qz] * uq[1][qz] + uq[2][qz] * uq[2][qz];
      const Real u_mag = fmax(sqrt(un2), Real(1e-12));
      const Real t1 = Real(2) * u_mag / hst, t2 = Real(4) * nu / (hst * hst);
      tauq[qz] = Real(1) / sqrt((Real)P.sdt2 + t1 * t1 + Real(9) * (t2 * t2));
    }
    double *const lrow = LIN && P.qd ? P.qd + qdp_base(brick, valid ? ci : 0, pa + 3 * pb) : nullptr;
    float *const lrowf = LIN && P.qdf ? P.qdf + qdp_base(brick, valid ? ci : 0, pa + 3 * pb) : nullptr;
// ... 283 lines not shown
    }
    backward(3, Z);
  }
  }
  __syncthreads();

  if constexpr (RST) {
    restrict_store();
  } else {
    if (P.ev) write_ev();
    else reduce_scatter(P.y, P.slab, true);
  }
}


bool pencil_enabled() {
  const char *e = std::getenv("GLS_PENCIL");
  return !(e && std::atoi(e) == 0);
}

template <typename Real, int MODE, bool FB = false>
hipError_t launch_pencil_t(const OpParams &P, const Tables1D &T, hipStream_t s) {
  const bool gen = P.srf || (MODE != MODE_JVQ && P.force_q);
  const int n_items = ((std::is_same<Real, double>::value || P.brick_cell0) && P.subset) ? P.subset_n : P.n_cells / 8;
  if (n_items <= 0) return hipSuccess;
  const int n_groups = (n_items + 2) / 3;
  PencilTab<Real> tab;
  for (int q = 0; q < 3; ++q) {
    tab.w[q] = (Real)T.w[q];
    for (int i = 0; i < 3; ++i) {
      tab.V[q][i] = (Real)T.V[q][i];
      tab.D[q][i] = (Real)T.D[q][i];
      tab.S[q][i] = (Real)T.S[q][i];
    }
    tab.xi[q] = (Real)T.xi[q];
  }
  if constexpr (std::is_same<Real, float>::value && MODE == MODE_JVQ && !FB) {
    if (P.oseen) {
      if (gen)
        hipLaunchKernelGGL((gls_pencil_kernel<float, MODE_JVQ, true, false, true>), dim3((unsigned)n_groups), dim3(256),
                           pencil_lds_bytes<float>(MODE), s, P, tab);
      else
        hipLaunchKernelGGL((gls_pencil_kernel<float, MODE_JVQ, false, false, true>), dim3((unsigned)n_groups),
                           dim3(256), pencil_lds_bytes<float>(MODE), s, P, tab);
      return hipGetLastError();
    }
  }
  if (gen)
    hipLaunchKernelGGL((gls_pencil_kernel<Real, MODE, true, FB>), dim3((unsigned)n_groups), dim3(256),
                       pencil_lds_bytes<Real>(MODE), s, P, tab);
  else
    hipLaunchKernelGGL((gls_pencil_kernel<Real, MODE, false, FB>), dim3((unsigned)n_groups), dim3(256),
                       pencil_lds_bytes<Real>(MODE), s, P, tab);
  return hipGetLastError();
}
hipError_t launch_pencil_jv(const OpParams &P, const Tables1D &T, hipStream_t s, bool f32) {
  if (P.n_probe > 0 || P.bricks || !(f32 ? (P.slabf != nullptr || P.slab != nullptr) : P.slab != nullptr))
    return hipErrorNotSupported;
  return f32 ? launch_pencil_t<float, MODE_JVQ>(P, T, s) : launch_pencil_t<double, MODE_JVQ>(P, T, s);
}
hipError_t launch_pencil_jv_restrict(const OpParams &P, const Tables1D &T, hipStream_t s) {
  if (P.n_probe > 0 || P.bricks || P.subset || P.brick_cell0 || P.srf || !P.slab || !P.rb || !P.qdf || P.jx || (P.jx0 && !P.jd) ||
      P.cube_nb1 <= 0 || (int64_t)P.cube_nb1 * P.cube_nb1 * P.cube_nb1 * 8 != P.n_cells)
    return hipErrorNotSupported;
  const int n_groups = (P.n_cells / 8 + 2) / 3;
  PencilTab<float> tab;
  for (int q = 0; q < 3; ++q) {
    tab.w[q] = (float)T.w[q];
    for (int i = 0; i < 3; ++i) {
      tab.V[q][i] = (float)T.V[q][i];
      tab.D[q][i] = (float)T.D[q][i];
      tab.S[q][i] = (float)T.S[q][i];
    }
    tab.xi[q] = (float)T.xi[q];
  }
  if (P.oseen)
    hipLaunchKernelGGL((gls_pencil_kernel<float, MODE_JVQ, false, false, true, true>), dim3((unsigned)n_groups), dim3(256),
                       pencil_lds_bytes<float>(MODE_JVQ), s, P, tab);
  else
    hipLaunchKernelGGL((gls_pencil_kernel<float, MODE_JVQ, false, false, false, true>), dim3((unsigned)n_groups), dim3(256),
                       pencil_lds_bytes<float>(MODE_JVQ), s, P, tab);
  return hipGetLastError();
}
hipError_t launch_pencil_residual(const OpParams &P, const Tables1D &T, hipStream_t s) {
  if (P.bricks || !P.slab || P.subset) return hipErrorNotSupported;
  return launch_pencil_t<double, MODE_RESIDUAL>(P, T, s);
}
hipError_t launch_pencil_reslin(const OpParams &P, const Tables1D &T, hipStream_t s) {
  if (P.bricks || P.subset || !P.qd || !P.y || !P.slab || !P.res_y || !P.res_slab) return hipErrorNotSupported;
  return launch_pencil_t<double, MODE_RESLIN>(P, T, s);
}
hipError_t launch_pencil_ev(int mode, const OpParams &P, const Tables1D &T, hipStream_t s, bool f32) {
  if ((!P.ev && mode != MODE_LIN) || P.y || !P.brick_cell0 || !P.subset || P.subset_n <= 0 || !P.qd || P.slab ||
      P.bricks || P.n_probe > 0 || P.rb || P.jx || P.jx0 || (f32 && (mode != MODE_JVQ || !P.qdf)))
    return hipErrorNotSupported;
  if (mode == MODE_JVQ && f32) return launch_pencil_t<float, MODE_JVQ, true>(P, T, s);
  if (mode == MODE_JVQ) return launch_pencil_t<double, MODE_JVQ>(P, T, s);
  if (mode == MODE_LIN) return launch_pencil_t<double, MODE_LIN>(P, T, s);
  return hipErrorNotSupported;
}
hipError_t launch_pencil_lin(const OpParams &P, const Tables1D &T, hipStream_t s) {
  if (P.bricks || (P.y && !P.slab) || P.subset || !P.qd) return hipErrorNotSupported;
  return launch_pencil_t<double, MODE_LIN>(P, T, s);
}

}
```

softx_2020_200_amd/csrc/gls_common.hpp:

```cpp
#pragma once
#include <hip/hip_runtime.h>

#include <cstdint>

namespace gls {

constexpr int kMaxNodes1D = 4;
constexpr int kMaxQ1D = 5;

constexpr int ipow(int b, int e) { return e == 0 ? 1 : b * ipow(b, e - 1); }

enum Mode { MODE_RESIDUAL = 0, MODE_JV = 1, MODE_DIAG = 2, MODE_LIN = 3, MODE_JVQ = 4,
            MODE_RESLIN = 5  };
constexpr int kQData = 16;

struct Tables1D {
  double V[kMaxQ1D][kMaxNodes1D];
  double D[kMaxQ1D][kMaxNodes1D];
  double S[kMaxQ1D][kMaxNodes1D];
  double Vp[kMaxQ1D][kMaxNodes1D];
  double Dp[kMaxQ1D][kMaxNodes1D];
  double w[kMaxQ1D];
  double xi[kMaxQ1D];
};

constexpr int kGeo = 22;
constexpr int kGeoX = 0, kGeoJxW = 3, kGeoJI = 4, kGeoG = 13, kGeoC = 19;

struct OpParams {
  int n_cells;
  int n_vnodes;
  int n_pnodes;
  int n_hist;
  const int32_t *cell_vnodes;
  const int32_t *cell_pnodes;
  const double *geo;
  const double *x0;
  const double *gq;
  const double *force_q;
  const uint8_t *vmask;
  const uint8_t *hmask;
  const int32_t *brick_cell0;
  const int32_t *cell_list;
  int cell_list_n;
  const double *u;
  const double *h1, *h2, *h3;
  const double *v;
  double *qd;
  float *qdf;
  int n_probe;
  int64_t probe_base;
  double *y;
  const int32_t *subset;
  int subset_n;
  double *ev;
  int64_t bv_stride;
  int64_t bev_stride;
  uint8_t *bact;
  const int32_t *work;
  int n_work;
  double *slab;
  float *slabf;
  double *jx;
  const double *jb, *jd;
  double jomega;
  const double *rb;
  double *jx0;
  double *res_y;
  double *res_slab;
  const int32_t *bricks;
  const uint16_t *ncolor;
  double *acc;
  int n_colors;
  int color;
  int color_off[17];
  double nu;
  double alpha[4];
  double alpha_jac;
  double sdt2;
  int srf;
  double omega[3];
  int oseen;
  double *cq;
  int cq_mode;
  int cube_nb1;
};

}
```

softx_2020_200_amd/csrc/gls_launch.hpp:

```cpp
#pragma once
#include "gls_common.hpp"

namespace gls {

hipError_t gather_element_vectors(double *y, const double *ev, const int64_t *voff, const int64_t *vslot, int64_t nv,
                                  const int64_t *poff, const int64_t *pslot, int64_t np, int dim, hipStream_t s);
hipError_t launch_cell_kernel(int dim, int k, int kp, int nq1d, int mode, const OpParams &P, const Tables1D &T,
                              hipStream_t s);
bool cell_kernel_supported(int dim, int k, int kp, int nq1d);
hipError_t launch_cell_sf_jv(int dim, int k, int kp, int nq1d, const OpParams &P, const Tables1D &T, hipStream_t s);
bool cell_sf_enabled();
int cell_kernel_cells_per_block(int dim, int k, int nq1d, bool probe = false);
hipError_t launch_brick_kernel(int k, int mode, const OpParams &P, const Tables1D &T, hipStream_t s);
size_t brick_qdata_size(int k, int n_cells);
hipError_t launch_brick_jv_f32(int k, const OpParams &P, const Tables1D &T, hipStream_t s);
hipError_t vec_to_f32(const double *a, float *b, int64_t n, hipStream_t s);
hipError_t vec_from_f32(const float *a, double *b, int64_t n, hipStream_t s);
hipError_t launch_pencil_jv(const OpParams &P, const Tables1D &T, hipStream_t s, bool f32);
hipError_t launch_pencil_jv_restrict(const OpParams &P, const Tables1D &T, hipStream_t s);
hipError_t launch_pencil_residual(const OpParams &P, const Tables1D &T, hipStream_t s);
hipError_t launch_pencil_lin(const OpParams &P, const Tables1D &T, hipStream_t s);
hipError_t launch_pencil_reslin(const OpParams &P, const Tables1D &T, hipStream_t s);
hipError_t launch_pencil_ev(int mode, const OpParams &P, const Tables1D &T, hipStream_t s, bool f32 = false);
bool pencil_enabled();
hipError_t launch_brick_wave(int k, int mode, const OpParams &P, const Tables1D &T, hipStream_t s);
hipError_t launch_brick_wave_jv_f32(int k, const OpParams &P, const Tables1D &T, hipStream_t s);
hipError_t launch_brick_wave_probe(int k, const OpParams &P, const Tables1D &T, int64_t j0, int nprobe, hipStream_t s);
size_t brick_wave_qdata_size(int k, int n_cells);

int brick_boundary_nodes(int k);
hipError_t brick_slab_sum(const double *slab, const int32_t *nodes, const int32_t *off, const int32_t *slots,
                          int64_t n_sum, int64_t n_vnodes, double *y, hipStream_t s);
hipError_t brick_slab_sum_ex(const double *slab, const float *slabf, const int32_t *nodes, const int32_t *off,
                             const int32_t *slots, int64_t n_sum, int64_t n_vnodes, double *y, const uint8_t *vmask,
                             const double *jb, const double *jd, double jomega, hipStream_t s,
                             const double *rb = nullptr);
hipError_t brick_slab_sum_cube(int k, int nb1, const double *slab, const float *slabf, int64_t n_vnodes, double *y,
                               const uint8_t *vmask, const double *jb, const double *jd, double jomega, hipStream_t s,
                               const double *rb = nullptr, double *x0 = nullptr);
hipError_t brick_restrict_sum_cube(int nb1, const double *ev, int64_t n_vnodes, double *bc, const uint8_t *vmask,
                                   hipStream_t s);
bool brick_fused_jacobi_supported(int k);
bool brick_colors_supported(int k);
bool brick_subset_supported(int k);
hipError_t launch_brick_probe(int k, const OpParams &P, const Tables1D &T, int64_t j0, int nprobe, hipStream_t s);

hipError_t vec_fill(double *x, int64_t n, double a, hipStream_t s);
hipError_t vec_copy(double *y, const double *x, int64_t n, hipStream_t s);
hipError_t vec_axpy(double *y, double a, const double *x, int64_t n, hipStream_t s);
hipError_t vec_axpby(double *y, double a, const double *x, double b, int64_t n, hipStream_t s);
hipError_t vec_scale(double *x, double a, int64_t n, hipStream_t s);
hipError_t vec_div(double *y, const double *x, const double *d, int64_t n, hipStream_t s);
hipError_t vec_multidot(const double *A, int64_t lda, int nk, const double *w, int64_t n, double *out,
                        double *work, hipStream_t s);
hipError_t vec_multidot2(const double *A, int64_t lda, int nk, const double *w, int64_t n1, int64_t off2, int64_t n2,
                         double *out, double *work, hipStream_t s);
hipError_t vec_pack_nodes(const double *x, const int32_t *nodes, int64_t m, int64_t voff, double *buf, hipStream_t s);
hipError_t vec_unpack_nodes(double *x, const int32_t *nodes, int64_t m, int64_t voff, const double *buf, int add,
                            hipStream_t s);
hipError_t vec_multiaxpy(double *w, const double *A, int64_t lda, int nk, const double *h, double sign, int64_t n,
                         hipStream_t s, bool zero_init = false);
hipError_t vec_waxpy(double *w, const double *y, double a, const double *x, int64_t n, hipStream_t s);
hipError_t vec_multiaxpy_dots(double *w, const double *A, int64_t lda, int nk, const double *h, double sign, int64_t n,
                              int64_t n1, int64_t off2, int64_t n2, bool dots, double scale, double *out,
                              double *work, hipStream_t s);
hipError_t vec_csr_gather_set(double *x, const double *src, const int64_t *dof, const int64_t *off,
                              const int64_t *master, const double *w, int64_t n, hipStream_t s);
hipError_t vec_copy_gather_set(double *x, const double *v, const uint8_t *dmask, int64_t n, const int64_t *dof,
                               const int64_t *off, const int64_t *master, const double *w, int64_t nl, hipStream_t s);
hipError_t vec_csr_condense(double *y, const int64_t *tm, const int64_t *toff, const int64_t *tdof, const double *tw,
                            int64_t n, hipStream_t s);
hipError_t vec_csr_spmv(double *y, const double *x, const int64_t *off, const int32_t *col, const double *w, int64_t n,
                        bool add, hipStream_t s, int lanes = 1);
hipError_t vec_gather_scale_set(double *y, const double *d, const double *v, const int64_t *idx, int64_t m,
                                hipStream_t s, const double *rb = nullptr);
hipError_t vec_set_const_indexed(double *x, const int32_t *idx, int64_t m, double a, hipStream_t s);
hipError_t csr_probe_extract(double *val, const int64_t *ent, const int32_t *row, int64_t m, const double *y,
                             hipStream_t s, bool add = false);
hipError_t csr_to_dense(double *A, const int64_t *rowp, const int32_t *col, const double *val, const int32_t *perm,
                        const int32_t *inv, int64_t n, hipStream_t s);
hipError_t vec_permute(double *out, const double *in, const int32_t *idx, int64_t n, int dir, hipStream_t s);
hipError_t probe_set_batched(double *V, int64_t n, const int32_t *dofs, const int32_t *pid, int p0, int64_t m,
                             hipStream_t s);
hipError_t probe_extract_batched(double *val, const int64_t *ent, const int32_t *row, const int32_t *pid, int p0,
                                 int64_t m, const double *Y, int64_t n, hipStream_t s);
hipError_t vec_csr_gather_set_b(double *x, const int64_t *dof, const int64_t *off, const int64_t *master,
                                const double *w, int64_t n, int nb, int64_t bs, hipStream_t s);
hipError_t vec_csr_condense_b(double *y, const int64_t *tm, const int64_t *toff, const int64_t *tdof, const double *tw,
                              int64_t n, int nb, int64_t bs, hipStream_t s);
hipError_t vec_gather_scale_set_b(double *y, const double *d, const double *v, const int64_t *idx, int64_t m, int nb,
                                  int64_t bs, hipStream_t s);
hipError_t gather_element_vectors_b(double *y, const double *ev, const int64_t *voff, const int64_t *vslot, int64_t nv,
                                    const int64_t *poff, const int64_t *pslot, int64_t np, int dim, int nb, int64_t ys,
                                    int64_t evs, const uint8_t *act, int64_t el, int cb, int nblk, hipStream_t s);
constexpr int kMaxGroupRows = 4;
constexpr int kIluMaxRow = 640;
constexpr int kIluCompactRow = 448;
hipError_t ilu_mc_factor(const int32_t *grow, const int32_t *color_groups, int n_colors, const int64_t *rowp,
                         const int32_t *col, double *val, const int64_t *lsp, const int64_t *didx, double boost_tol,
                         double boost_val, const int64_t *moff, const uint16_t *map, bool compact, double *rdiag,
                         hipStream_t s);
hipError_t ilu_mc_factor_map(int64_t n, const int64_t *rowp, const int32_t *col, const int64_t *lsp,
                             const int64_t *didx, const int64_t *moff, uint16_t *map, hipStream_t s);
constexpr int kGroupDesc = 24;
hipError_t ilu_mc_solve(const int64_t *gdesc, const int32_t *color_groups, int n_colors, const int32_t *col,
                        const double *val, const double *b, double *y, double *x, const uint8_t *waves_lower,
                        const uint8_t *waves_upper, hipStream_t s);
hipError_t vec_pack_dofs(const double *x, const int32_t *dofs, int64_t m, double *buf, hipStream_t s);
hipError_t vec_unpack_dofs(double *x, const int32_t *dofs, int64_t m, const double *buf, hipStream_t s);
hipError_t vec_add_dofs_ordered(double *x, const int32_t *u, const int32_t *off, const int32_t *slot, int64_t n,
                                const double *buf, hipStream_t s);
hipError_t vec_add_nodes_ordered(double *x, const int32_t *u, const int32_t *off, const int32_t *slot, int64_t n,
                                 int64_t voff, const double *buf, hipStream_t s);
hipError_t csr_diag_perturb(double *val, const int64_t *didx, int64_t n, double athresh, double rthresh, hipStream_t s);
hipError_t vec_set_const_indexed64(double *x, const int64_t *idx, int64_t m, double a, hipStream_t s);
hipError_t vec_add_pos_ordered(double *x, const int64_t *u, const int32_t *off, const int32_t *slot, int64_t n,
                               const double *buf, hipStream_t s);
hipError_t vec_set_indexed(double *y, const int64_t *idx, const double *vals, int64_t m, hipStream_t s);
int multidot_work_size();

struct KellyTables {
  int nq;
// ... 64 lines not shown
```

softx_2020_200_amd/native.py:

```python
from __future__ import annotations

import ctypes as C
import os

import numpy as np

HERE = os.path.dirname(os.path.abspath(__file__))
LIB_PATH = os.environ.get("GLS_NATIVE_LIB") or os.path.join(HERE, "libgls_native.so")

GLS_OK, GLS_EINVAL, GLS_EHIP, GLS_ENOMEM, GLS_ENOCONV, GLS_EIO, GLS_ECOMM = 0, -1, -2, -3, -4, -5, -6

SCHEMES = {
    "steady": 0, "bdf1": 1, "bdf2": 2, "bdf3": 3, "sdirk2": 4, "sdirk2_1": 5, "sdirk2_2": 6,
    "sdirk3": 7, "sdirk3_1": 8, "sdirk3_2": 9, "sdirk3_3": 10,
}

EXPORTS = [
    "gls_last_error", "gls_version", "gls_create", "gls_destroy", "gls_set_stream", "gls_n_dofs", "gls_set_force",
    "gls_set_viscosity", "gls_set_time", "gls_set_state", "gls_residual", "gls_jacobian_apply",
    "gls_jacobian_apply_f32",
    "gls_jacobian_diagonal", "gls_set_dirichlet", "gls_apply_dirichlet", "gls_solve_linear", "gls_newton_solve",
    "gls_bdf_coefficients", "gls_sdirk_coefficients", "gls_newton_selftest", "gls_mesh_hyper_cube_sizes",
    "gls_mesh_hyper_cube", "gls_timing_reset", "gls_timing_get", "gls_timing_enable", "gls_uses_brick_kernels",
    "gls_part_create", "gls_part_sizes", "gls_part_get", "gls_part_destroy", "gls_dist_attach", "gls_dist_import", "gls_rccl_unique_id", "gls_rccl_create", "gls_rccl_destroy", "gls_rccl_info", "gls_mg_smoother_apply", "gls_mg_attach_replica",
    "gls_dist_attach_rccl",
    "gls_mg_attach", "gls_mg_detach", "gls_mg_set_coarse_replica", "gls_residual_and_diagonal", "gls_octree_set_periodic", "gls_ilu_attach", "gls_ilu_detach", "gls_ilu_info", "gls_ilu_matrix", "gls_ilu_factors", "gls_ilu_set_options", "gls_iluk_pattern", "gls_cuthill_mckee", "gls_section_timing", "gls_section_get", "gls_dist_attach_dofs", "gls_dist_attach_dofs_rccl", "gls_gpart_create", "gls_gpart_sizes", "gls_gpart_get", "gls_gpart_map_dofs", "gls_gpart_destroy", "gls_dpart_create", "gls_set_lattice", "gls_apply_preconditioner", "gls_mg_transfer",
    "gls_mg_residual_restrict",
    "gls_prm_parse", "gls_prm_get", "gls_prm_n_entries", "gls_prm_entry", "gls_prm_destroy",
    "gls_expr_create", "gls_expr_n_components", "gls_expr_eval", "gls_expr_destroy",
    "gls_vtu_write", "gls_pvtu_write", "gls_pvd_write",
    "gls_set_hanging", "gls_mesh_refined_create", "gls_mesh_refined_destroy", "gls_octree_create", "gls_octree_destroy", "gls_octree_info",
    "gls_octree_cells", "gls_octree_adapt", "gls_octree_prepare", "gls_octree_mesh", "gls_octree_mesh_destroy", "gls_octree_transfer", "gls_octree_faces", "gls_kelly_estimate_faces",
    "gls_kelly_estimate", "gls_refine_fixed_number", "gls_mesh_refined_interpolate", "gls_refine_pd", "gls_refine_coarsen_pd",
    "gls_freeze_jacobian", "gls_skip_newton_selftest", "gls_quadrature_points",
    "gls_umesh_generate", "gls_umesh_read_gmsh", "gls_umesh_set_manifold", "gls_umesh_boundary_manifold",
    "gls_umesh_refine_global", "gls_umesh_info", "gls_umesh_destroy", "gls_umesh_fe_space", "gls_fe_space_destroy",
    "gls_fe_space_transfer", "gls_umesh_prepare", "gls_umesh_adapt", "gls_umesh_set_periodic", "gls_fe_space_kelly_faces",
    "gls_kelly_estimate_mapped", "gls_fe_space_boundary_normals", "gls_fe_space_boundary_normal_sets",
    "gls_octree_coarsen_to", "gls_octree_mg_transfer", "gls_mg_attach_transfers", "gls_umesh_coarsen_to",
    "gls_fe_space_mg_transfer", "gls_forest_bricks",
    "gls_fe_space_boundary_faces", "gls_boundary_plan_create", "gls_boundary_plan_destroy", "gls_boundary_loads",
    "gls_flow_diagnostics", "gls_time_control_create", "gls_time_control_destroy", "gls_time_control_integrate",
    "gls_time_control_set_cfl", "gls_time_control_get", "gls_time_control_is_output_iteration",
    "gls_output_plan_create", "gls_output_plan_destroy", "gls_output_fields", "gls_vtu_write_device",
]


class GLSError(RuntimeError):
    pass


class MeshDesc(C.Structure):
    _fields_ = [
        ("dim", C.c_int), ("k", C.c_int), ("kp", C.c_int), ("nq1d", C.c_int), ("n_cells", C.c_int),
        ("n_vnodes", C.c_int), ("n_pnodes", C.c_int),
        ("cell_vnodes", C.POINTER(C.c_int32)), ("cell_pnodes", C.POINTER(C.c_int32)),
        ("cell_x0", C.POINTER(C.c_double)), ("cell_h", C.POINTER(C.c_double)),
        ("vnode_mask", C.POINTER(C.c_uint8)),
        ("viscosity", C.c_double), ("srf", C.c_int), ("omega", C.c_double * 3),
        ("force_q", C.POINTER(C.c_double)),
        ("map_degree", C.c_int), ("cell_support", C.POINTER(C.c_double)),
    ]


class FESpace(C.Structure):
    _fields_ = [("dim", C.c_int), ("k", C.c_int), ("kp", C.c_int),
                ("n_cells", C.c_int64), ("n_vnodes", C.c_int64), ("n_pnodes", C.c_int64),
                ("cell_vnodes", C.POINTER(C.c_int32)), ("cell_pnodes", C.POINTER(C.c_int32)),
                ("vnode_x", C.POINTER(C.c_double)), ("pnode_x", C.POINTER(C.c_double)),
                ("vnode_bid", C.POINTER(C.c_uint32)), ("pnode_bid", C.POINTER(C.c_uint32)),
                ("cell_support", C.POINTER(C.c_double)), ("cell_mapping", C.POINTER(C.c_int32)),
                ("cell_measure", C.POINTER(C.c_double)), ("volume", C.c_double),
                ("cell_level", C.POINTER(C.c_int32)),
                ("n_vhang", C.c_int64), ("vhang_node", C.POINTER(C.c_int64)), ("vhang_off", C.POINTER(C.c_int64)),
                ("vhang_master", C.POINTER(C.c_int64)), ("vhang_w", C.POINTER(C.c_double)),
                ("n_phang", C.c_int64), ("phang_node", C.POINTER(C.c_int64)), ("phang_off", C.POINTER(C.c_int64)),
                ("phang_master", C.POINTER(C.c_int64)), ("phang_w", C.POINTER(C.c_double)),
                ("impl_", C.c_void_p)]


class LinearParams(C.Structure):
    _fields_ = [("max_iterations", C.c_int), ("restart", C.c_int), ("relative_residual", C.c_double),
                ("minimum_residual", C.c_double), ("iterations", C.c_int), ("final_residual", C.c_double),
                ("method", C.c_int), ("orthogonalization", C.c_int), ("true_residual", C.c_int)]


LIN_METHODS = {"gmres": 0, "bicgstab": 1}
ORTHO = {"gram": 0, "cgs2": 1}


class MGParams(C.Structure):
    _fields_ = [("n_levels", C.c_int), ("levels", C.POINTER(C.c_void_p)), ("pre_smooth", C.c_int),
                ("post_smooth", C.c_int), ("coarse_sweeps", C.c_int), ("omega", C.c_double),
                ("coarse_omega", C.c_double), ("coarse_direct", C.c_int), ("mixed_precision", C.c_int),
                ("level_sweeps", C.POINTER(C.c_int)), ("smoother", C.c_int), ("smoother_operator", C.c_int)]


class TimeControlParams(C.Structure):
    _fields_ = [("dt", C.c_double), ("time_end", C.c_double), ("adapt", C.c_int), ("max_cfl", C.c_double),
                ("scaling", C.c_double), ("output_control", C.c_int), ("output_frequency", C.c_int),
                ("output_time", C.c_double)]


OUTPUT_CONTROL = {"iteration": 0, "time": 1}


class RefinedMesh(C.Structure):
    _fields_ = [("dim", C.c_int), ("k", C.c_int), ("kp", C.c_int),
                ("n_cells", C.c_int64), ("n_vnodes", C.c_int64), ("n_pnodes", C.c_int64),
                ("cell_vnodes", C.POINTER(C.c_int32)), ("cell_pnodes", C.POINTER(C.c_int32)),
                ("cell_level", C.POINTER(C.c_int32)),
                ("cell_x0", C.POINTER(C.c_double)), ("cell_h", C.POINTER(C.c_double)),
                ("vnode_x", C.POINTER(C.c_double)), ("pnode_x", C.POINTER(C.c_double)),
                ("n_vhang", C.c_int64), ("vhang_node", C.POINTER(C.c_int64)), ("vhang_off", C.POINTER(C.c_int64)),
                ("vhang_master", C.POINTER(C.c_int64)), ("vhang_w", C.POINTER(C.c_double)),
                ("n_phang", C.c_int64), ("phang_node", C.POINTER(C.c_int64)), ("phang_off", C.POINTER(C.c_int64)),
                ("phang_master", C.POINTER(C.c_int64)), ("phang_w", C.POINTER(C.c_double)),
                ("impl_", C.c_void_p)]


class NewtonParams(C.Structure):
    _fields_ = [("tolerance", C.c_double), ("max_iterations", C.c_int), ("verbosity", C.c_int),
                ("lin", LinearParams), ("newton_iterations", C.c_int), ("linear_iterations", C.c_int),
                ("residual_evaluations", C.c_int), ("final_residual", C.c_double),
                ("solver", C.c_int), ("skip_iterations", C.c_int), ("is_initial_step", C.c_int),
                ("force_matrix_renewal", C.c_int), ("linear_failures", C.c_int)]


_lib = None


def load():
    global _lib
    if _lib is not None:
        return _lib
    if not os.path.exists(LIB_PATH):
        raise GLSError("HIP extension %s is missing — run `python -m softx_2020_200_amd.build` "
                       "(or __graft_entry__.build()); there is no CPU fallback" % LIB_PATH)
    L = C.CDLL(LIB_PATH)
    vp, d, i64 = C.c_void_p, C.POINTER(C.c_double), C.c_int64
    L.gls_last_error.restype = C.c_char_p
    L.gls_version.restype = C.c_char_p
    L.gls_create.argtypes = [C.POINTER(MeshDesc), C.POINTER(vp)]
    L.gls_destroy.argtypes = [vp]
    L.gls_set_stream.argtypes = [vp, vp]
    L.gls_n_dofs.argtypes = [vp, C.POINTER(i64)]
    L.gls_set_force.argtypes = [vp, d]
    L.gls_set_viscosity.argtypes = [vp, C.c_double]
    L.gls_set_time.argtypes = [vp, C.c_int, d]
    L.gls_set_state.argtypes = [vp, vp, vp, vp, vp]
    L.gls_residual.argtypes = [vp, vp]
    L.gls_jacobian_apply.argtypes = [vp, vp, vp]
    L.gls_jacobian_apply_f32.argtypes = [vp, vp, vp]
    L.gls_jacobian_diagonal.argtypes = [vp, vp]
    L.gls_residual_and_diagonal.argtypes = [vp, vp, vp]
    L.gls_set_dirichlet.argtypes = [vp, i64, C.POINTER(i64), d]
    L.gls_apply_dirichlet.argtypes = [vp, vp]
    L.gls_solve_linear.argtypes = [vp, vp, vp, C.POINTER(LinearParams)]
    L.gls_newton_solve.argtypes = [vp, vp, vp, vp, vp, C.POINTER(NewtonParams)]
    L.gls_bdf_coefficients.argtypes = [C.c_int, d, C.c_int, d]
    L.gls_sdirk_coefficients.argtypes = [C.c_int, C.c_double, d]
    L.gls_newton_selftest.argtypes = [d]
    L.gls_skip_newton_selftest.argtypes = [C.c_int, d]
    L.gls_freeze_jacobian.argtypes = [vp, C.c_int]
    L.gls_mesh_hyper_cube_sizes.argtypes = [C.c_int] * 5 + [C.POINTER(i64)] * 3
    L.gls_mesh_hyper_cube.argtypes = [C.c_int] * 4 + [C.c_double, C.c_double, C.c_int,
                                                      C.POINTER(C.c_int32), C.POINTER(C.c_int32), d, d]
    L.gls_timing_reset.argtypes = [vp]
    L.gls_timing_get.argtypes = [vp, C.c_int, d, C.POINTER(i64)]
    L.gls_timing_enable.argtypes = [vp, C.c_int]
    L.gls_uses_brick_kernels.argtypes = [vp]
    L.gls_mg_attach.argtypes = [vp, C.POINTER(MGParams)]
    L.gls_mg_detach.argtypes = [vp]
    L.gls_mg_set_coarse_replica.argtypes = [vp, vp, i64, C.POINTER(i64)]
    L.gls_mg_attach_transfers.argtypes = [vp, C.POINTER(MGParams), C.POINTER(C.POINTER(i64)),
                                          C.POINTER(C.POINTER(C.c_int32)), C.POINTER(C.POINTER(C.c_double)),
                                          C.POINTER(C.POINTER(i64))]
    L.gls_octree_coarsen_to.argtypes = [vp, C.c_int, C.POINTER(vp)]
    L.gls_umesh_coarsen_to.argtypes = [vp, C.c_int, C.POINTER(vp)]
    L.gls_forest_bricks.argtypes = [vp]
    L.gls_fe_space_mg_transfer.argtypes = [C.POINTER(FESpace), C.POINTER(FESpace), C.POINTER(i64), vp, vp, vp, vp]
    L.gls_octree_mg_transfer.argtypes = [C.POINTER(RefinedMesh), C.POINTER(RefinedMesh), C.POINTER(i64), vp, vp, vp, vp]
    L.gls_set_lattice.argtypes = [vp, C.c_int, C.POINTER(i64)]
    L.gls_apply_preconditioner.argtypes = [vp, vp, vp]
    L.gls_mg_smoother_apply.argtypes = [vp, vp, vp]
    L.gls_mg_attach_replica.argtypes = [vp, C.POINTER(MGParams), vp, C.POINTER(C.c_int64), C.POINTER(C.c_int32),
                                        C.POINTER(C.c_double), C.POINTER(C.c_int64)]
    L.gls_mg_transfer.argtypes = [vp, C.c_int, C.c_int, vp, vp]
    L.gls_mg_residual_restrict.argtypes = [vp, C.c_int, vp, vp, vp, C.POINTER(C.c_int)]
    P64 = C.POINTER(i64)
    L.gls_set_hanging.argtypes = [vp, i64, P64, P64, P64, d]
    L.gls_mesh_refined_create.argtypes = [C.c_int, C.c_int, C.c_int, C.c_int, C.c_double, C.c_double,
                                          C.POINTER(C.c_int32), C.POINTER(C.POINTER(RefinedMesh))]
    L.gls_mesh_refined_destroy.argtypes = [C.POINTER(RefinedMesh)]
    L.gls_kelly_estimate.argtypes = [vp, vp, C.c_int, vp]
    L.gls_refine_fixed_number.argtypes = [i64, C.POINTER(C.c_float), C.c_double, C.POINTER(C.c_int32)]
    L.gls_refine_pd.argtypes = [i64, C.POINTER(C.c_float), C.c_int, C.c_int, C.c_double, i64,
                                C.POINTER(C.c_int32), C.POINTER(C.c_double)]
    L.gls_mesh_refined_interpolate.argtypes = [C.POINTER(RefinedMesh), C.c_int, C.c_double, C.c_double,
                                               C.POINTER(C.c_double), C.POINTER(C.c_double)]
    L.gls_quadrature_points.argtypes = [vp, d]
    L.gls_umesh_generate.argtypes = [C.c_int, C.c_char_p, C.c_char_p, C.POINTER(vp)]
    L.gls_umesh_read_gmsh.argtypes = [C.c_int, C.c_char_p, C.POINTER(vp)]
    L.gls_umesh_set_manifold.argtypes = [vp, C.c_int, C.c_int, d, d]
    L.gls_umesh_boundary_manifold.argtypes = [vp, C.c_int, C.c_int]
    L.gls_umesh_refine_global.argtypes = [vp, C.c_int]
    L.gls_umesh_info.argtypes = [vp, C.POINTER(i64), C.POINTER(i64), d]
    L.gls_umesh_destroy.argtypes = [vp]
    L.gls_umesh_destroy.restype = None
    L.gls_umesh_fe_space.argtypes = [vp, C.c_int, C.c_int, C.c_int, C.c_int, C.POINTER(C.c_int32),
                                     C.POINTER(C.POINTER(FESpace))]
    L.gls_fe_space_destroy.argtypes = [C.POINTER(FESpace)]
    L.gls_fe_space_transfer.argtypes = [C.POINTER(FESpace), C.POINTER(FESpace), d, d]
    pi32 = C.POINTER(C.c_int32)
    L.gls_umesh_prepare.argtypes = [vp, pi32, pi32]
    L.gls_umesh_adapt.argtypes = [vp, pi32, pi32]
    L.gls_umesh_set_periodic.argtypes = [vp, C.c_int, pi32]
    L.gls_fe_space_kelly_faces.argtypes = [C.POINTER(FESpace), C.c_int, C.POINTER(i64), pi32, pi32, d, d, d, d]
    L.gls_fe_space_boundary_normals.argtypes = [C.POINTER(FESpace), C.c_int, d]
    L.gls_fe_space_boundary_normal_sets.argtypes = [C.POINTER(FESpace), C.c_int, C.POINTER(C.c_int32), d]
    L.gls_kelly_estimate_mapped.argtypes = [vp, vp, C.c_int, i64, C.c_int, pi32, pi32, d, d, d, d, vp]
    L.gls_fe_space_boundary_faces.argtypes = [C.POINTER(FESpace), C.c_int, C.POINTER(i64), pi32, pi32, pi32, d, d, d, d, d]
    L.gls_boundary_plan_create.argtypes = [vp, i64, C.c_int, pi32, pi32, d, d, d, d, d, C.c_int, C.POINTER(vp)]
    L.gls_boundary_plan_destroy.argtypes = [vp]
    L.gls_boundary_loads.argtypes = [vp, vp, vp, C.c_double, d, d, d]
    L.gls_flow_diagnostics.argtypes = [vp, vp, C.c_double, d]
    L.gls_output_plan_create.argtypes = [vp, C.POINTER(MeshDesc), C.c_int, C.POINTER(vp)]
    L.gls_output_plan_destroy.argtypes = [vp]
    L.gls_output_fields.argtypes = [vp, vp, vp, d, d, d, d, d, d]
    L.gls_vtu_write_device.argtypes = [vp, vp, vp, C.c_char_p, C.c_int, C.c_int]
    L.gls_time_control_create.argtypes = [C.POINTER(TimeControlParams), C.POINTER(vp)]
    L.gls_time_control_destroy.argtypes = [vp]
    L.gls_time_control_destroy.restype = None
    L.gls_time_control_integrate.argtypes = [vp]
    L.gls_time_control_set_cfl.argtypes = [vp, C.c_double]
    L.gls_time_control_get.argtypes = [vp, C.POINTER(C.c_int), d, d, d]
    L.gls_time_control_is_output_iteration.argtypes = [vp]
    _lib = L
    return L


def check(rc, what=""):
    if rc < 0:
        msg = load().gls_last_error().decode()
        raise GLSError("%s failed (%d): %s" % (what, rc, msg))
    return rc


def _dp(a):
    return a.ctypes.data_as(C.POINTER(C.c_double)) if a is not None else C.POINTER(C.c_double)()


def mesh_desc(mesh, srf=False, omega=(0.0, 0.0, 0.0)):
    get = mesh.get if isinstance(mesh, dict) else lambda key, default=None: getattr(mesh, key, default)
    dim, k, kp = int(get("dim")), int(get("k")), int(get("kp"))
    keep = []

    def arr(a, dt):
        if a is None:
            return None
        keep.append(np.ascontiguousarray(a, dtype=dt))
        return keep[-1]

    cv = arr(get("cell_vnodes"), np.int32)
    cp = arr(get("cell_pnodes"), np.int32) if kp != k else None
    md = int(get("map_degree") or 0) if get("cell_support") is not None else 0
    D = MeshDesc()
    D.dim, D.k, D.kp, D.nq1d = dim, k, kp, 0
    D.n_cells, D.n_vnodes, D.n_pnodes = cv.shape[0], int(get("n_vnodes")), int(get("n_pnodes"))
    D.cell_vnodes = cv.ctypes.data_as(C.POINTER(C.c_int32))
    D.cell_pnodes = cp.ctypes.data_as(C.POINTER(C.c_int32)) if cp is not None else C.POINTER(C.c_int32)()
    if md:
# ... 570 lines not shown
        self._mg_replica = (replica, keep)

    def set_coarse_replica(self, replica, local_to_replica):
        m = np.ascontiguousarray(local_to_replica, dtype=np.int64)
        check(self.L.gls_mg_set_coarse_replica(self.h, replica.h, len(m), m.ctypes.data_as(C.POINTER(C.c_int64))),
              "gls_mg_set_coarse_replica")
        self._coarse_replica = replica

    def mg_smoother_apply(self, v, out=None):
        out = self.zeros() if out is None else out
        check(self.L.gls_mg_smoother_apply(self.h, _ptr(v), _ptr(out)), "gls_mg_smoother_apply")
        return out

    def apply_preconditioner(self, v, out=None):
        out = self.zeros() if out is None else out
        check(self.L.gls_apply_preconditioner(self.h, _ptr(v), _ptr(out)), "gls_apply_preconditioner")
        return out

    def kelly_estimate(self, sol, variable=0, out=None):
        import torch
        out = torch.empty(self.n_cells, dtype=torch.float64, device=sol.device) if out is None else out
        check(self.L.gls_kelly_estimate(self.h, _ptr(sol), int(variable), _ptr(out)), "gls_kelly_estimate")
        return out

    def kelly_estimate_faces(self, sol, variable, faces, out=None):
        import torch
        fa, fb, fd, ra, rb = faces
        out = torch.empty(self.n_cells, dtype=torch.float64, device=sol.device) if out is None else out
        self.L.gls_kelly_estimate_faces.argtypes = [C.c_void_p, C.c_void_p, C.c_int, C.c_int64] + [C.c_void_p] * 6
        check(self.L.gls_kelly_estimate_faces(self.h, _ptr(sol), int(variable), len(fa), fa.ctypes.data, fb.ctypes.data,
                                              fd.ctypes.data, ra.ctypes.data, rb.ctypes.data, _ptr(out)),
              "gls_kelly_estimate_faces")
        return out

    def kelly_estimate_mapped(self, sol, variable, faces, out=None):
        import torch
        out = torch.empty(self.n_cells, dtype=torch.float64, device=sol.device) if out is None else out
        f = {k: np.ascontiguousarray(v) for k, v in faces.items() if isinstance(v, np.ndarray)}
        p32 = lambda a: a.ctypes.data_as(C.POINTER(C.c_int32))
        check(self.L.gls_kelly_estimate_mapped(self.h, _ptr(sol), int(variable), len(f["ca"]), int(faces["nqf"]),
                                               p32(f["ca"]), p32(f["cb"]), _dp(f["xi"]), _dp(f["g"]), _dp(f["jxw"]),
                                               _dp(f["diam"]), _ptr(out)), "gls_kelly_estimate_mapped")
        return out

    def flow_diagnostics(self, sol, dt):
        out = np.zeros(4)
        check(self.L.gls_flow_diagnostics(self.h, _ptr(sol), float(dt), _dp(out)), "gls_flow_diagnostics")
        return out

    def boundary_loads(self, faces, slots, n_slots, sol, viscosity, cor):
        f = {k: np.ascontiguousarray(v) for k, v in faces.items() if isinstance(v, np.ndarray)}
        sl = np.ascontiguousarray(slots, dtype=np.int32)
        if sl.shape != (len(f["cell"]),):
            raise GLSError("boundary_loads: one slot per face")
        cor = np.ascontiguousarray(cor, dtype=np.float64)
        if cor.shape != (int(n_slots), 3):
            raise GLSError("boundary_loads: cor is [n_slots][3]")
        p32 = lambda a: a.ctypes.data_as(C.POINTER(C.c_int32))
        plan = C.c_void_p()
        check(self.L.gls_boundary_plan_create(self.h, len(sl), int(faces["nqf"]), p32(f["cell"]), p32(sl), _dp(f["xi"]),
                                              _dp(f["jinv"]), _dp(f["normal"]), _dp(f["jxw"]), _dp(f["xq"]),
                                              int(n_slots), C.byref(plan)), "gls_boundary_plan_create")
        force, torque = np.zeros((int(n_slots), 3)), np.zeros((int(n_slots), 3))
        try:
            check(self.L.gls_boundary_loads(self.h, plan, _ptr(sol), float(viscosity), _dp(cor), _dp(force), _dp(torque)),
                  "gls_boundary_loads")
        finally:
            self.L.gls_boundary_plan_destroy(plan)
        return force, torque

    def output_plan(self, mesh, subdivision=1, srf=False, omega=(0.0, 0.0, 0.0)):
        return OutputPlan(self, mesh, subdivision, srf, omega)

    def mg_transfer(self, level, direction, v, out):
        check(self.L.gls_mg_transfer(self.h, int(level), int(direction), _ptr(v), _ptr(out)), "gls_mg_transfer")
        return out

    def mg_residual_restrict(self, level, x, b, out):
        fused = C.c_int(0)
        check(self.L.gls_mg_residual_restrict(self.h, int(level), _ptr(x), _ptr(b), _ptr(out), C.byref(fused)),
              "gls_mg_residual_restrict")
        return out, bool(fused.value)

    def set_lattice(self, n1d, local_to_global):
        l2g = np.ascontiguousarray(local_to_global, dtype=np.int64)
        check(self.L.gls_set_lattice(self.h, int(n1d), l2g.ctypes.data_as(C.POINTER(C.c_int64))), "gls_set_lattice")

    def detach_multigrid(self):
        check(self.L.gls_mg_detach(self.h), "gls_mg_detach")
        self._mg_levels = None

    def attach_ilu(self, athresh=1e-8, rthresh=1.0, fill=0, block_dofs=0, ordering="cm"):
        self.L.gls_ilu_set_options.argtypes = [C.c_void_p, C.c_int, C.c_int64]
        check(self.L.gls_ilu_set_options(self.h, {"cm": 0, "multicolor": 1}[ordering], int(block_dofs)),
              "gls_ilu_set_options")
        self.L.gls_ilu_attach.argtypes = [C.c_void_p, C.c_int, C.c_double, C.c_double]
        check(self.L.gls_ilu_attach(self.h, int(fill), float(athresh), float(rthresh)), "gls_ilu_attach")
        nnz, npr = C.c_int64(), C.c_int()
        self.L.gls_ilu_info.argtypes = [C.c_void_p, C.POINTER(C.c_int64), C.POINTER(C.c_int)]
        check(self.L.gls_ilu_info(self.h, C.byref(nnz), C.byref(npr)), "gls_ilu_info")
        return nnz.value, npr.value

    def ilu_factors(self):
        import scipy.sparse as sp
        nnz, _ = C.c_int64(), C.c_int()
        self.L.gls_ilu_info.argtypes = [C.c_void_p, C.POINTER(C.c_int64), C.POINTER(C.c_int)]
        check(self.L.gls_ilu_info(self.h, C.byref(nnz), C.byref(_)), "gls_ilu_info")
        perm = np.zeros(self.n_dofs, dtype=np.int32)
        rowp = np.zeros(self.n_dofs + 1, dtype=np.int32)
        col = np.zeros(nnz.value, dtype=np.int32)
        val = np.zeros(nnz.value)
        self.L.gls_ilu_factors.argtypes = [C.c_void_p] * 5
        check(self.L.gls_ilu_factors(self.h, perm.ctypes.data, rowp.ctypes.data, col.ctypes.data, val.ctypes.data),
              "gls_ilu_factors")
        return perm, sp.csr_matrix((val, col, rowp), shape=(self.n_dofs, self.n_dofs))

    def ilu_matrix(self):
        import scipy.sparse as sp
        nnz, _ = C.c_int64(), C.c_int()
        self.L.gls_ilu_info.argtypes = [C.c_void_p, C.POINTER(C.c_int64), C.POINTER(C.c_int)]
        check(self.L.gls_ilu_info(self.h, C.byref(nnz), C.byref(_)), "gls_ilu_info")
        rowp = np.zeros(self.n_dofs + 1, dtype=np.int32)
        col = np.zeros(nnz.value, dtype=np.int32)
        val = np.zeros(nnz.value)
        self.L.gls_ilu_matrix.argtypes = [C.c_void_p, C.c_void_p, C.c_void_p, C.c_void_p]
        check(self.L.gls_ilu_matrix(self.h, rowp.ctypes.data, col.ctypes.data, val.ctypes.data), "gls_ilu_matrix")
        return sp.csr_matrix((val, col, rowp), shape=(self.n_dofs, self.n_dofs))

    def detach_ilu(self):
        self.L.gls_ilu_detach.argtypes = [C.c_void_p]
        check(self.L.gls_ilu_detach(self.h), "gls_ilu_detach")

    def timing(self, enable=True):
        check(self.L.gls_timing_enable(self.h, 1 if enable else 0), "gls_timing_enable")
        check(self.L.gls_timing_reset(self.h), "gls_timing_reset")

    def timing_get(self, which):
        ms, n = C.c_double(), C.c_int64()
        check(self.L.gls_timing_get(self.h, which, C.byref(ms), C.byref(n)), "gls_timing_get")
        return ms.value, n.value


MANIFOLD_TYPES = {"flat": 0, "spherical": 1, "cylindrical": 2}


class OutputPlan:

    def __init__(self, ctx, mesh, subdivision, srf=False, omega=(0.0, 0.0, 0.0)):
        self.ctx, self.L = ctx, ctx.L
        D, keep = mesh_desc(mesh, srf, omega)
        self.dim, self.srf = D.dim, bool(srf)
        self.n_points = D.n_cells * (int(subdivision) + 1) ** D.dim
        h = C.c_void_p()
        check(self.L.gls_output_plan_create(ctx.h, C.byref(D), int(subdivision), C.byref(h)), "gls_output_plan_create")
        self.h = h

    def close(self):
        if getattr(self, "h", None):
            self.L.gls_output_plan_destroy(self.h)
            self.h = None

    def __del__(self):
        try:
            self.close()
        except Exception:
            pass
# ... 238 lines not shown
```

Before: 12.46 nonlinear_iters/s.

## Fuse multigrid Q2 prolongation into first post-smoothing pencil Jacobi sweep

Adds a PRO variant of the FP32 pencil J·v kernel. It computes the Q2 prolongation of the coarse correction inside the kernel's node gather, tensor-product line by line in LDS, and adds it to x on the fly. The kernel writes the prolonged start values to a side buffer that the cube slab-sum Jacobi update reads. This removes the separate prolong-add pass, along with its extra read and write of the fine vector, before the first post-smoothing sweep. In exchange it uses more LDS and more complex index logic, and it only applies under strict eligibility conditions (Q2, cube lattice, FP32 smoother, two-pass taps).

Result: faster. 12.71 nonlinear_iters/s (median of 6 runs) (+2.0%).

```diff
diff --git a/include/gls_native.h b/include/gls_native.h
--- a/include/gls_native.h
+++ b/include/gls_native.h
@@ -115,6 +115,8 @@
 int gls_mg_smoother_apply(gls_ctx *ctx, const double *v, double *y);
 int gls_mg_transfer(gls_ctx *ctx, int level, int direction, const double *in, double *out);
 int gls_mg_residual_restrict(gls_ctx *ctx, int level, const double *x, const double *b, double *bc, int *fused);
+int gls_mg_prolong_smooth(gls_ctx *ctx, int level, const double *xc, double *x, const double *b, double omega,
+                          int *fused);
 int gls_set_lattice(gls_ctx *ctx, int n1d, const int64_t *local_to_global);
 int gls_mg_detach(gls_ctx *ctx);
 int gls_mg_set_coarse_replica(gls_ctx *ctx, gls_ctx *replica, int64_t n_local, const int64_t *local_to_replica);
diff --git a/softx_2020_200_amd/csrc/gls_api.cpp b/softx_2020_200_amd/csrc/gls_api.cpp
--- a/softx_2020_200_amd/csrc/gls_api.cpp
+++ b/softx_2020_200_amd/csrc/gls_api.cpp
@@ -1018,11 +1018,12 @@
 }
 
 hipError_t slab_sum_ex(gls_ctx *g, const double *slab, const float *slabf, double *y, const uint8_t *vmask,
-                       const double *jb, const double *jd, double omega, const double *rb, double *x0 = nullptr) {
+                       const double *jb, const double *jd, double omega, const double *rb, double *x0 = nullptr,
+                       const double *xs = nullptr) {
   if (g->cube_nb1 > 0)
     return gls::brick_slab_sum_cube(g->k, g->cube_nb1, slab, slabf, g->n_vnodes, y, vmask, jb, jd, omega, g->stream, rb,
-                                    x0);
-  if (x0) return hipErrorInvalidValue;
+                                    x0, xs);
+  if (x0 || xs) return hipErrorInvalidValue;
   return gls::brick_slab_sum_ex(slab, slabf, g->sum_nodes.p, g->sum_off.p, g->sum_slots.p, (int64_t)g->sum_nodes.n,
                                 g->n_vnodes, y, vmask, jb, jd, omega, g->stream, rb);
 }
@@ -1856,11 +1857,14 @@
   HIP_TRY(gls::vec_axpy(x, 1.0, z, g->n_dofs, g->stream));
   return GLS_OK;
 }
-int smoother_sweep(gls_ctx *g, double *x, const double *b, double *y, double omega, double *z = nullptr) {
-  if (z && g->ilu.on && !g->ilu.probe_only) return ilu_sweep(g, x, b, y, z);
+int smoother_sweep(gls_ctx *g, double *x, const double *b, double *y, double omega, double *z = nullptr,
+                   const double *pxc = nullptr) {
   const bool nofuse = std::getenv("GLS_MG_NO_FUSE") != nullptr;
   const bool brick = g->use_brick && g->use_qdata && (g->use_colors || brick_slab(g)) && !g->dist.on &&
                      !g->hang.on && gls::brick_fused_jacobi_supported(g->k);
+  if (pxc && ((z && g->ilu.on && !g->ilu.probe_only) || nofuse || !brick || !g->smooth_f32 || g->use_colors || g->cube_nb1 <= 0))
+    return set_err(GLS_EINVAL, "fused prolongation not applicable");
+  if (z && g->ilu.on && !g->ilu.probe_only) return ilu_sweep(g, x, b, y, z);
   if (nofuse || !brick) {
     GLS_TRY(smoother_apply(g, x, y));
     HIP_TRY(gls::mg_jacobi_update(x, b, y, g->diag.p, omega, g->n_dofs, 0, g->stream));
@@ -1887,8 +1891,12 @@
     P.qdf = g->qdata32.p;
     P.oseen = g->smooth_oseen ? 1 : 0;
     P.slabf = P.slab && slab_f32() ? reinterpret_cast<float *>(P.slab) : nullptr;
+    P.pxc = pxc;
+    P.pxp = pxc ? y : nullptr;
+    P.cube_nb1 = g->cube_nb1;
     TimedLaunch t(g, 4);
-    HIP_TRY(gls::launch_brick_jv_f32(g->k, P, g->tables, g->stream));
+    HIP_TRY(pxc ? gls::launch_pencil_jv_prolong(P, g->tables, g->stream)
+                : gls::launch_brick_jv_f32(g->k, P, g->tables, g->stream));
   } else {
     P.qd = g->qdata.p;
     TimedLaunch t(g, 1);
@@ -1896,7 +1904,7 @@
   }
   if (g->use_colors) return GLS_OK;
   TimedLaunch t(g, 5);
-  HIP_TRY(slab_sum_ex(g, P.slab, P.slabf, x, g->vmask.p, b, g->diag.p, omega, nullptr));
+  HIP_TRY(slab_sum_ex(g, P.slab, P.slabf, x, g->vmask.p, b, g->diag.p, omega, nullptr, nullptr, pxc ? y : nullptr));
   return GLS_OK;
 }
 }
@@ -2621,6 +2629,23 @@
   return GLS_OK;
 }
 
+bool mg_fused_prolong_ok(gls_ctx *c, int l) {
+  auto &mg = c->mg;
+  if (l < 0 || l + 1 >= (int)mg.lev.size() || mg.csr || mg.boxed || (size_t)l >= mg.taps.size() || !mg_prolong_add_ok(c, l))
+    return false;
+  const char *e = std::getenv("GLS_MG_FUSE_PROLONG");
+  if (e && std::atoi(e) == 0) return false;
+  gls_ctx *g = mg.lev[(size_t)l], *h = mg.lev[(size_t)l + 1];
+  const auto &T = *mg.taps[(size_t)l];
+  const int64_t nc1 = 2 * (int64_t)g->cube_nb1 + 1;
+  const bool ilu_smooth = mg.ilu_smooth && g->ilu.on && !g->ilu.probe_only;
+  return T.two_pass && T.q2_brick && mg.lpost[(size_t)l] >= 1 && !ilu_smooth && g->smooth_f32 && g->use_brick &&
+         g->use_qdata && !g->use_colors && !g->dist.on && !g->hang.on && !g->oct.on && g->k == 2 && g->cube_nb1 > 0 &&
+         g->cube_nb1 < 1024 && g->use_slab && brick_slab(g) && !g->srf && gls::pencil_enabled() &&
+         gls::brick_fused_jacobi_supported(g->k) && !h->dist.on && !h->hang.on && h->cube_nb1 > 0 &&
+         g->cube_nb1 == 2 * h->cube_nb1 && h->n_vnodes == nc1 * nc1 * nc1 && g->stream == c->stream;
+}
+
 bool coarse_graph_eligible(gls_ctx *c, gls_ctx *g, const double *b, const double *x) {
   const int l = (int)c->mg.lev.size() - 1;
   return !c->mg.cgraph_failed && !c->mg.boxed && !g->dist.on && !g->hang.on && g->use_brick && g->use_qdata &&
@@ -2876,14 +2901,17 @@
     HIP_TRY(gls::vec_set_indexed(bc, h->con_dofs.p, nullptr, (int64_t)h->con_dofs.n, s));
   }
   GLS_TRY(mg_vcycle(c, l + 1, bc, xc));
-  if (mg_prolong_add_ok(c, l)) {
+  const bool pro = mg_fused_prolong_ok(c, l);
+  if (pro) {
+  } else if (mg_prolong_add_ok(c, l)) {
     GLS_TRY(mg_prolong(c, l, xc, x, true));
   } else {
     GLS_TRY(mg_prolong(c, l, xc, y));
     HIP_TRY(gls::vec_set_indexed(y, g->con_dofs.p, nullptr, (int64_t)g->con_dofs.n, s));
     HIP_TRY(gls::vec_axpy(x, 1.0, y, n, s));
   }
-  for (int it = 0; it < mg.lpost[(size_t)l]; ++it) GLS_TRY(smoother_sweep(g, x, b, y, mg.omega, zs));
+  for (int it = 0; it < mg.lpost[(size_t)l]; ++it)
+    GLS_TRY(smoother_sweep(g, x, b, y, mg.omega, zs, pro && it == 0 ? xc : nullptr));
   return GLS_OK;
 }
 
@@ -3134,6 +3162,31 @@
   GLS_TRY(mg_restrict(c, level, y, bc));
   HIP_TRY(gls::vec_set_indexed(bc, h->con_dofs.p, nullptr, (int64_t)h->con_dofs.n, c->stream));
   return GLS_OK;
+}
+
+int gls_mg_prolong_smooth(gls_ctx *c, int level, const double *xc, double *x, const double *b, double omega, int *fused) {
+  GLS_TRY(check_ctx(c));
+  auto &mg = c->mg;
+  if (!mg.on) return set_err(GLS_EINVAL, "gls_mg_prolong_smooth: no multigrid attached");
+  if (level < 0 || level + 1 >= (int)mg.lev.size() || !xc || !x || !b || x == b || omega < 0.0)
+    return set_err(GLS_EINVAL, "gls_mg_prolong_smooth: bad level / pointers / omega");
+  GLS_TRY(mg_prepare(c));
+  gls_ctx *g = mg.lev[(size_t)level];
+  const bool f = mg_fused_prolong_ok(c, level);
+  if (fused) *fused = f ? 1 : 0;
+  double *y = mgbuf(c, level, MB_Y);
+  double *zs = mg.ilu_smooth && g->ilu.on && !g->ilu.probe_only ? mgbuf(c, level, MB_BOX) : nullptr;
+  double *xcw = mgbuf(c, level + 1, MB_X);
+  if (xcw != xc) HIP_TRY(gls::vec_copy(xcw, xc, mg.lev[(size_t)level + 1]->n_dofs, c->stream));
+  if (f) return smoother_sweep(g, x, b, y, omega, zs, xcw);
+  if (mg_prolong_add_ok(c, level)) {
+    GLS_TRY(mg_prolong(c, level, xcw, x, true));
+  } else {
+    GLS_TRY(mg_prolong(c, level, xcw, y));
+    HIP_TRY(gls::vec_set_indexed(y, g->con_dofs.p, nullptr, (int64_t)g->con_dofs.n, c->stream));
+    HIP_TRY(gls::vec_axpy(x, 1.0, y, g->n_dofs, c->stream));
+  }
+  return smoother_sweep(g, x, b, y, omega, zs);
 }
 
 namespace {
diff --git a/softx_2020_200_amd/csrc/gls_brick_common.hpp b/softx_2020_200_amd/csrc/gls_brick_common.hpp
--- a/softx_2020_200_amd/csrc/gls_brick_common.hpp
+++ b/softx_2020_200_amd/csrc/gls_brick_common.hpp
@@ -20,6 +20,22 @@
   return n - before;
 }
 
+__device__ __forceinline__ int morton_compact3(unsigned v) {
+  v &= 0x09249249u;
+  v = (v ^ (v >> 2)) & 0x030c30c3u;
+  v = (v ^ (v >> 4)) & 0x0300f00fu;
+  v = (v ^ (v >> 8)) & 0xff0000ffu;
+  return (int)((v ^ (v >> 16)) & 0x3ffu);
+}
+
+__device__ __forceinline__ void q2_prolong_line(double c0, double c1, double c2, double (&o)[5]) {
+  o[0] = c0;
+  o[1] = fma(-0.125, c2, fma(0.75, c1, 0.375 * c0));
+  o[2] = c1;
+  o[3] = fma(0.375, c2, fma(0.75, c1, -0.125 * c0));
+  o[4] = c2;
+}
+
 __device__ __forceinline__ void wave_sync() {
 #ifdef GLS_WAVE_SYNC_DRAIN
   asm volatile("s_waitcnt lgkmcnt(0)" ::: "memory");
diff --git a/softx_2020_200_amd/csrc/gls_brick_kernels.hip b/softx_2020_200_amd/csrc/gls_brick_kernels.hip
--- a/softx_2020_200_amd/csrc/gls_brick_kernels.hip
+++ b/softx_2020_200_amd/csrc/gls_brick_kernels.hip
@@ -1106,12 +1106,13 @@
     m |= (((x >> b) & 1u) << (3 * b)) | (((y >> b) & 1u) << (3 * b + 1)) | (((z >> b) & 1u) << (3 * b + 2));
   return m;
 }
-template <typename S, bool J, int K>
+template <typename S, bool J, int K, bool XS = false>
 __global__ void __launch_bounds__(256) k_slab_sum_cube(const S *__restrict__ slab, int nb1, int64_t voff,
                                                        double *__restrict__ y, const uint8_t *__restrict__ vmask,
                                                        const double *__restrict__ jb, const double *__restrict__ jd,
                                                        double jomega, const double *__restrict__ rb,
-                                                       double *__restrict__ x0) {
+                                                       double *__restrict__ x0, const double *__restrict__ xs) {
+  static_assert(!XS || J, "start values: fused Jacobi sweep");
   constexpr int BN = 2 * K + 1, P2 = 2 * K, NBND = BN * BN * BN - (BN - 2) * (BN - 2) * (BN - 2);
   const int NX = P2 * nb1 + 1;
   int bx = blockIdx.x, Z = blockIdx.y;
@@ -1204,7 +1205,7 @@
     const unsigned m = vmask ? vmask[node] : 0u;
 #pragma unroll
     for (int f = 0; f < 4; ++f) {
-      const double x = y[gi[f]], dd = jd[gi[f]];
+      const double x = XS ? xs[gi[f]] : y[gi[f]], dd = jd[gi[f]];
       y[gi[f]] = x + jomega * (jb[gi[f]] - ((f < 3 && ((m >> f) & 1u)) ? dd * x : s[f])) / dd;
     }
   } else if (rb) {
@@ -1221,19 +1222,26 @@
 }
 hipError_t brick_slab_sum_cube(int k, int nb1, const double *slab, const float *slabf, int64_t n_vnodes, double *y,
                                const uint8_t *vmask, const double *jb, const double *jd, double jomega, hipStream_t s,
-                               const double *rb, double *x0) {
+                               const double *rb, double *x0, const double *xs) {
   if (nb1 <= 0 || (k != 1 && k != 2)) return hipErrorInvalidValue;
   if (x0 && (!rb || !jd || jb)) return hipErrorInvalidValue;
+  if (xs && (k != 2 || !jb || !jd || xs == y)) return hipErrorInvalidValue;
   const int NX = 2 * k * nb1 + 1;
   const dim3 g((unsigned)(((int64_t)NX * NX + 255) / 256), (unsigned)NX), b(256);
   const int64_t voff = 3 * n_vnodes;
-#define GLS_SLAB_CUBE(KK)                                                                                                   \
+  if (xs) {
+    if (slabf) hipLaunchKernelGGL((k_slab_sum_cube<float, true, 2, true>), g, b, 0, s, slabf, nb1, voff, y, vmask, jb, jd, jomega, rb, x0, xs);
+    else hipLaunchKernelGGL((k_slab_sum_cube<double, true, 2, true>), g, b, 0, s, slab, nb1, voff, y, vmask, jb, jd, jomega, rb, x0, xs);
+    return hipGetLastError();
+  }
+  const double *const no_xs = nullptr;
+#define GLS_SLAB_CUBE(KK)                                                                                                  \
   if (slabf) {                                                                                                              \
-    if (jb) hipLaunchKernelGGL((k_slab_sum_cube<float, true, KK>), g, b, 0, s, slabf, nb1, voff, y, vmask, jb, jd, jomega, rb, x0);  \
-    else hipLaunchKernelGGL((k_slab_sum_cube<float, false, KK>), g, b, 0, s, slabf, nb1, voff, y, vmask, jb, jd, jomega, rb, x0);   \
+    if (jb) hipLaunchKernelGGL((k_slab_sum_cube<float, true, KK>), g, b, 0, s, slabf, nb1, voff, y, vmask, jb, jd, jomega, rb, x0, no_xs);  \
+    else hipLaunchKernelGGL((k_slab_sum_cube<float, false, KK>), g, b, 0, s, slabf, nb1, voff, y, vmask, jb, jd, jomega, rb, x0, no_xs);   \
   } else {                                                                                                                  \
-    if (jb) hipLaunchKernelGGL((k_slab_sum_cube<double, true, KK>), g, b, 0, s, slab, nb1, voff, y, vmask, jb, jd, jomega, rb, x0); \
-    else hipLaunchKernelGGL((k_slab_sum_cube<double, false, KK>), g, b, 0, s, slab, nb1, voff, y, vmask, jb, jd, jomega, rb, x0);  \
+    if (jb) hipLaunchKernelGGL((k_slab_sum_cube<double, true, KK>), g, b, 0, s, slab, nb1, voff, y, vmask, jb, jd, jomega, rb, x0, no_xs); \
+    else hipLaunchKernelGGL((k_slab_sum_cube<double, false, KK>), g, b, 0, s, slab, nb1, voff, y, vmask, jb, jd, jomega, rb, x0, no_xs);  \
   }
   if (k == 1) {
     GLS_SLAB_CUBE(1)
diff --git a/softx_2020_200_amd/csrc/gls_brick_pencil.hip b/softx_2020_200_amd/csrc/gls_brick_pencil.hip
--- a/softx_2020_200_amd/csrc/gls_brick_pencil.hip
+++ b/softx_2020_200_amd/csrc/gls_brick_pencil.hip
@@ -13,6 +13,9 @@
 #endif
 #ifndef GLS_PENCIL_NT
 #define GLS_PENCIL_NT 0
+#endif
+#ifndef GLS_PENCIL_PRO_XP_LDS
+#define GLS_PENCIL_PRO_XP_LDS 1
 #endif
 #ifndef GLS_PENCIL_WPE32
 #define GLS_PENCIL_WPE32 4
@@ -55,11 +58,12 @@
   Real V[3][3], D[3][3], S[3][3], w[3], xi[3];
 };
 
-template <typename Real, int MODE, bool GEN, bool FOREST = false, bool OS = false, bool RST = false>
+template <typename Real, int MODE, bool GEN, bool FOREST = false, bool OS = false, bool RST = false, bool PRO = false>
 __global__ void __launch_bounds__(256, (std::is_same<Real, float>::value ? GLS_PENCIL_WPE32 : GLS_PENCIL_WPE64))
     gls_pencil_kernel(const OpParams P, const PencilTab<Real> T) {
   static_assert(!OS || (MODE == MODE_JVQ && std::is_same<Real, float>::value), "Oseen operator: FP32 J.v only");
   static_assert(!RST || (MODE == MODE_JVQ && std::is_same<Real, float>::value && !FOREST), "restriction: FP32 J.v on the cube");
+  static_assert(!PRO || (MODE == MODE_JVQ && std::is_same<Real, float>::value && !FOREST && !RST), "prolongation: FP32 J.v on the cube");
   using C = PencilCfg<Real, MODE == MODE_JVQ>;
   constexpr bool RL = MODE == MODE_RESLIN, RES = MODE == MODE_RESIDUAL || RL, LIN = MODE == MODE_LIN || RL;
   constexpr bool ST = RES || LIN;
@@ -71,6 +75,7 @@
   constexpr int CS = C::CS;
   Real *const sO = sS + C::WAVES * C::CPW * CS;
   int *const sNode = reinterpret_cast<int *>(sO + C::CPG * C::OC);
+  double *const sXP = reinterpret_cast<double *>(sNode + C::BPG * BN3P);
   __shared__ Real sRow[3 * 16];
 
   const int tid = threadIdx.x, lane = tid & 63, wave = tid >> 6;
@@ -107,7 +112,95 @@
                                                           : reinterpret_cast<const Real *>(P.qdf);
     qrow = base + qdp_base(brick, valid ? ci : 0, pa + 3 * pb);
   }
-  for (int t = tid; t < C::BPG * BN3; t += C::THREADS) {
+  double *const dPX = reinterpret_cast<double *>(sO), *const dPY = dPX + C::BPG * 4 * 45;
+  double *const dPZ = reinterpret_cast<double *>(sS);
+  if constexpr (PRO) {
+    static_assert((C::BPG * NF * FB) % 2 == 0 && (C::WAVES * C::CPW * CS) % 2 == 0 && (C::CPG * C::OC + C::BPG * BN3P) % 2 == 0 &&
+                      C::WAVES * C::CPW * CS >= 2 * C::BPG * 4 * BN3 && C::CPG * C::OC >= 2 * C::BPG * 4 * (45 + 75),
+                  "prolongation scratch in LDS");
+    static_assert(C::BPG * BN3 <= 2 * C::THREADS, "two brick nodes per thread");
+    int gn[2];
+    unsigned gm[2];
+    double gx[2][4];
+#pragma unroll
+    for (int it = 0; it < 2; ++it) {
+      const int t = tid + it * C::THREADS, bi = t / BN3, n = t - BN3 * bi;
+      gn[it] = -1;
+      if (bi < nbg) {
+        const int X = n % BN, Y = (n / BN) % BN, Z = n / (BN * BN);
+        const int cx = min(X / 2, 1), cy = min(Y / 2, 1), cz = min(Z / 2, 1);
+        const int a = (X - 2 * cx) + 3 * ((Y - 2 * cy) + 3 * (Z - 2 * cz));
+        const int node = P.cell_vnodes[(cell0(brick_of(bi)) + cx + 2 * cy + 4 * cz) * 27 + a];
+        gn[it] = node;
+        gx[it][0] = P.v[(int64_t)node * 3];
+        gx[it][1] = P.v[(int64_t)node * 3 + 1];
+        gx[it][2] = P.v[(int64_t)node * 3 + 2];
+        gx[it][3] = P.v[voff + node];
+        gm[it] = P.vmask ? P.vmask[node] : 0u;
+      }
+    }
+    const int ncx = 2 * P.cube_nb1 + 1;
+    double o[5];
+    for (int t = tid; t < nbg * 36; t += C::THREADS) {
+      const int bf = t / 9, jk = t - 9 * bf, bi = bf >> 2, f = bf & 3, j = jk % 3, k = jk / 3;
+      const unsigned bk = (unsigned)brick_of(bi);
+      const int64_t cn = 2 * morton_compact3(bk) +
+                         (int64_t)ncx * ((2 * morton_compact3(bk >> 1) + j) + (int64_t)ncx * (2 * morton_compact3(bk >> 2) + k));
+      const double *c = f < 3 ? P.pxc + cn * 3 + f : P.pxc + (int64_t)3 * ncx * ncx * ncx + cn;
+      const int st = f < 3 ? 3 : 1;
+      q2_prolong_line(c[0], c[st], c[2 * st], o);
+#pragma unroll
+      for (int X = 0; X < 5; ++X) dPX[bf * 45 + 5 * jk + X] = o[X];
+    }
+    __syncthreads();
+    for (int t = tid; t < nbg * 60; t += C::THREADS) {
+      const int bf = t / 15, r = t - 15 * bf, k = r / 5, X = r - 5 * k;
+      const double *x = dPX + bf * 45 + 15 * k + X;
+      q2_prolong_line(x[0], x[5], x[10], o);
+#pragma unroll
+      for (int Y = 0; Y < 5; ++Y) dPY[bf * 75 + 25 * k + 5 * Y + X] = o[Y];
+    }
+    __syncthreads();
+    for (int t = tid; t < nbg * 100; t += C::THREADS) {
+      const int bf = t / 25, yx = t - 25 * bf;
+      const double *y = dPY + bf * 75 + yx;
+      q2_prolong_line(y[0], y[25], y[50], o);
+#pragma unroll
+      for (int Z = 0; Z < 5; ++Z) dPZ[bf * BN3 + 25 * Z + yx] = o[Z];
+    }
+    __syncthreads();
+#pragma unroll
+    for (int it = 0; it < 2; ++it) {
+      if (gn[it] < 0) continue;
+      const int t = tid + it * C::THREADS, bi = t / BN3, n = t - BN3 * bi, node = gn[it];
+      const int X = n % BN, Y = (n / BN) % BN, Z = n / (BN * BN);
+      const double *pz = dPZ + bi * 4 * BN3 + n;
+      const double v0 = gx[it][0] + pz[0], v1 = gx[it][1] + pz[BN3], v2 = gx[it][2] + pz[2 * BN3], vp = gx[it][3] + pz[3 * BN3];
+      if (GLS_PENCIL_PRO_XP_LDS && X > 0 && X < BN - 1 && Y > 0 && Y < BN - 1 && Z > 0 && Z < BN - 1) {
+        typedef double d2 __attribute__((ext_vector_type(2)));
+        d2 *xo = reinterpret_cast<d2 *>(sXP + (bi * 27 + (X - 1) + 3 * ((Y - 1) + 3 * (Z - 1))) * 4);
+        xo[0] = d2{v0, v1};
+        xo[1] = d2{v2, vp};
+      } else {
+        const unsigned bk = (unsigned)brick_of(bi);
+        const int top = P.cube_nb1 - 1;
+        if ((X < BN - 1 || morton_compact3(bk) == top) && (Y < BN - 1 || morton_compact3(bk >> 1) == top) &&
+            (Z < BN - 1 || morton_compact3(bk >> 2) == top)) {
+          P.pxp[(int64_t)node * 3] = v0;
+          P.pxp[(int64_t)node * 3 + 1] = v1;
+          P.pxp[(int64_t)node * 3 + 2] = v2;
+          P.pxp[voff + node] = vp;
+        }
+      }
+      Real *b = sB + bi * NF * FB + X + SY * Y + SZ * Z;
+      b[0] = (gm[it] & 1u) ? Real(0) : (Real)v0;
+      b[FB] = (gm[it] & 2u) ? Real(0) : (Real)v1;
+      b[2 * FB] = (gm[it] & 4u) ? Real(0) : (Real)v2;
+      b[3 * FB] = (Real)vp;
+      sNode[bi * BN3P + n] = node;
+    }
+  }
+  for (int t = tid; t < (PRO ? 0 : C::BPG * BN3); t += C::THREADS) {
     const int bi = t / BN3, n = t % BN3;
     if (bi >= nbg) break;
     const int brick = brick_of(bi);
@@ -302,7 +395,8 @@
 #pragma unroll
           for (int f = 0; f < 4; ++f) {
             const bool con = f < 3 && ((m >> f) & 1u);
-            const double x = P.jx[gi[f]], dd = P.jd[gi[f]];
+            const double x = !PRO ? P.jx[gi[f]] : GLS_PENCIL_PRO_XP_LDS ? sXP[(rb_ * 27 + (Xn - 1) + 3 * ((Yn - 1) + 3 * (Zn - 1))) * 4 + f] : P.pxp[gi[f]];
+            const double dd = P.jd[gi[f]];
             P.jx[gi[f]] = x + P.jomega * (P.jb[gi[f]] - (con ? dd * x : (double)s[f])) / dd;
           }
         } else if (fused && P.rb) {
@@ -347,13 +441,6 @@
       c0 = r0 + (0.375 * r1 - 0.125 * r3);
       c1 = r2 + 0.75 * (r1 + r3);
       c2 = r4 + (0.375 * r3 - 0.125 * r1);
-    };
-    auto compact3 = [](unsigned v) {
-      v &= 0x09249249u;
-      v = (v ^ (v >> 2)) & 0x030c30c3u;
-      v = (v ^ (v >> 4)) & 0x0300f00fu;
-      v = (v ^ (v >> 8)) & 0xff0000ffu;
-      return (int)((v ^ (v >> 16)) & 0x3ffu);
     };
     static_assert((C::BPG * NF * FB + C::WAVES * C::CPW * CS) % 2 == 0 && C::BPG * NF * FB + C::WAVES * C::CPW * CS >= 2 * (C::BPG * 4 * (BN3 + 45)) &&
                       C::CPG * C::OC >= 2 * C::BPG * 4 * 75, "restriction scratch in LDS");
@@ -385,8 +472,8 @@
       }
       const int node = sNode[rb_ * BN3P + n];
       const int top = P.cube_nb1 - 1;
-      const bool own = (Xn < BN - 1 || compact3((unsigned)bk) == top) && (Yn < BN - 1 || compact3((unsigned)bk >> 1) == top) &&
-                       (Zn < BN - 1 || compact3((unsigned)bk >> 2) == top);
+      const bool own = (Xn < BN - 1 || morton_compact3((unsigned)bk) == top) && (Yn < BN - 1 || morton_compact3((unsigned)bk >> 1) == top) &&
+                       (Zn < BN - 1 || morton_compact3((unsigned)bk >> 2) == top);
       const unsigned m = P.vmask ? P.vmask[node] : 0u;
       double r[4] = {-(double)s[0], -(double)s[1], -(double)s[2], -(double)s[3]};
       if (own) {
@@ -836,6 +923,31 @@
                        pencil_lds_bytes<float>(MODE_JVQ), s, P, tab);
   return hipGetLastError();
 }
+hipError_t launch_pencil_jv_prolong(const OpParams &P, const Tables1D &T, hipStream_t s) {
+  if (P.n_probe > 0 || P.bricks || P.subset || P.brick_cell0 || P.srf || !(P.slab || P.slabf) || !P.qdf || !P.pxc || !P.pxp || P.pxp == P.jx || !P.jx ||
+      P.jx != P.v || !P.jb || !P.jd || P.rb || P.jx0 || P.ev || P.cube_nb1 <= 0 || P.cube_nb1 > 1023 ||
+      (int64_t)P.cube_nb1 * P.cube_nb1 * P.cube_nb1 * 8 != P.n_cells)
+    return hipErrorNotSupported;
+  const int n_groups = (P.n_cells / 8 + 2) / 3;
+  PencilTab<float> tab;
+  for (int q = 0; q < 3; ++q) {
+    tab.w[q] = (float)T.w[q];
+    for (int i = 0; i < 3; ++i) {
+      tab.V[q][i] = (float)T.V[q][i];
+      tab.D[q][i] = (float)T.D[q][i];
+      tab.S[q][i] = (float)T.S[q][i];
+    }
+    tab.xi[q] = (float)T.xi[q];
+  }
+  const size_t lds = pencil_lds_bytes<float>(MODE_JVQ) + (GLS_PENCIL_PRO_XP_LDS ? sizeof(double) * PencilCfg<float, true>::BPG * 27 * 4 : 0);
+  if (P.oseen)
+    hipLaunchKernelGGL((gls_pencil_kernel<float, MODE_JVQ, false, false, true, false, true>), dim3((unsigned)n_groups),
+                       dim3(256), lds, s, P, tab);
+  else
+    hipLaunchKernelGGL((gls_pencil_kernel<float, MODE_JVQ, false, false, false, false, true>), dim3((unsigned)n_groups),
+                       dim3(256), lds, s, P, tab);
+  return hipGetLastError();
+}
 hipError_t launch_pencil_residual(const OpParams &P, const Tables1D &T, hipStream_t s) {
   if (P.bricks || !P.slab || P.subset) return hipErrorNotSupported;
   return launch_pencil_t<double, MODE_RESIDUAL>(P, T, s);
diff --git a/softx_2020_200_amd/csrc/gls_common.hpp b/softx_2020_200_amd/csrc/gls_common.hpp
--- a/softx_2020_200_amd/csrc/gls_common.hpp
+++ b/softx_2020_200_amd/csrc/gls_common.hpp
@@ -84,6 +84,8 @@
   double *cq;
   int cq_mode;
   int cube_nb1;
+  const double *pxc;
+  double *pxp;
 };
 
 }
diff --git a/softx_2020_200_amd/csrc/gls_launch.hpp b/softx_2020_200_amd/csrc/gls_launch.hpp
--- a/softx_2020_200_amd/csrc/gls_launch.hpp
+++ b/softx_2020_200_amd/csrc/gls_launch.hpp
@@ -18,6 +18,7 @@
 hipError_t vec_from_f32(const float *a, double *b, int64_t n, hipStream_t s);
 hipError_t launch_pencil_jv(const OpParams &P, const Tables1D &T, hipStream_t s, bool f32);
 hipError_t launch_pencil_jv_restrict(const OpParams &P, const Tables1D &T, hipStream_t s);
+hipError_t launch_pencil_jv_prolong(const OpParams &P, const Tables1D &T, hipStream_t s);
 hipError_t launch_pencil_residual(const OpParams &P, const Tables1D &T, hipStream_t s);
 hipError_t launch_pencil_lin(const OpParams &P, const Tables1D &T, hipStream_t s);
 hipError_t launch_pencil_reslin(const OpParams &P, const Tables1D &T, hipStream_t s);
@@ -37,7 +38,8 @@
                              const double *rb = nullptr);
 hipError_t brick_slab_sum_cube(int k, int nb1, const double *slab, const float *slabf, int64_t n_vnodes, double *y,
                                const uint8_t *vmask, const double *jb, const double *jd, double jomega, hipStream_t s,
-                               const double *rb = nullptr, double *x0 = nullptr);
+                               const double *rb = nullptr, double *x0 = nullptr,
+                               const double *xs = nullptr);
 hipError_t brick_restrict_sum_cube(int nb1, const double *ev, int64_t n_vnodes, double *bc, const uint8_t *vmask,
                                    hipStream_t s);
 bool brick_fused_jacobi_supported(int k);
diff --git a/softx_2020_200_amd/native.py b/softx_2020_200_amd/native.py
--- a/softx_2020_200_amd/native.py
+++ b/softx_2020_200_amd/native.py
@@ -25,7 +25,7 @@
     "gls_part_create", "gls_part_sizes", "gls_part_get", "gls_part_destroy", "gls_dist_attach", "gls_dist_import", "gls_rccl_unique_id", "gls_rccl_create", "gls_rccl_destroy", "gls_rccl_info", "gls_mg_smoother_apply", "gls_mg_attach_replica",
     "gls_dist_attach_rccl",
     "gls_mg_attach", "gls_mg_detach", "gls_mg_set_coarse_replica", "gls_residual_and_diagonal", "gls_octree_set_periodic", "gls_ilu_attach", "gls_ilu_detach", "gls_ilu_info", "gls_ilu_matrix", "gls_ilu_factors", "gls_ilu_set_options", "gls_iluk_pattern", "gls_cuthill_mckee", "gls_section_timing", "gls_section_get", "gls_dist_attach_dofs", "gls_dist_attach_dofs_rccl", "gls_gpart_create", "gls_gpart_sizes", "gls_gpart_get", "gls_gpart_map_dofs", "gls_gpart_destroy", "gls_dpart_create", "gls_set_lattice", "gls_apply_preconditioner", "gls_mg_transfer",
-    "gls_mg_residual_restrict",
+    "gls_mg_residual_restrict", "gls_mg_prolong_smooth",
     "gls_prm_parse", "gls_prm_get", "gls_prm_n_entries", "gls_prm_entry", "gls_prm_destroy",
     "gls_expr_create", "gls_expr_n_components", "gls_expr_eval", "gls_expr_destroy",
     "gls_vtu_write", "gls_pvtu_write", "gls_pvd_write",
@@ -188,6 +188,7 @@
                                         C.POINTER(C.c_double), C.POINTER(C.c_int64)]
     L.gls_mg_transfer.argtypes = [vp, C.c_int, C.c_int, vp, vp]
     L.gls_mg_residual_restrict.argtypes = [vp, C.c_int, vp, vp, vp, C.POINTER(C.c_int)]
+    L.gls_mg_prolong_smooth.argtypes = [vp, C.c_int, vp, vp, vp, C.c_double, C.POINTER(C.c_int)]
     P64 = C.POINTER(i64)
     L.gls_set_hanging.argtypes = [vp, i64, P64, P64, P64, d]
     L.gls_mesh_refined_create.argtypes = [C.c_int, C.c_int, C.c_int, C.c_int, C.c_double, C.c_double,
@@ -924,6 +925,12 @@
               "gls_mg_residual_restrict")
         return out, bool(fused.value)
 
+    def mg_prolong_smooth(self, level, xc, x, b, omega):
+        fused = C.c_int(0)
+        check(self.L.gls_mg_prolong_smooth(self.h, int(level), _ptr(xc), _ptr(x), _ptr(b), float(omega),
+                                           C.byref(fused)), "gls_mg_prolong_smooth")
+        return x, bool(fused.value)
+
     def set_lattice(self, n1d, local_to_global):
         l2g = np.ascontiguousarray(local_to_global, dtype=np.int64)
         check(self.L.gls_set_lattice(self.h, int(n1d), l2g.ctypes.data_as(C.POINTER(C.c_int64))), "gls_set_lattice")
```
